# yjxiong/action-detection

Measured on NVIDIA H100. Metric: proposals/sec (9-seg BNInception SSN fwd+bwd), higher is better.
Workload: dtype f32 via split f16 operands (hi+lo, 3 wgmma MMAs per product) / f32 accumulate; f32 storage

## Files before the change

action-detection_b200/csrc/common.cuh:

```cuda
#pragma once
#include <cuda_fp16.h>
#include <cuda_runtime.h>
#include <stdint.h>

#include <atomic>
#include <string>

namespace ssnb {

struct View {
  void* base = nullptr;
  int H = 0, W = 0, C = 0, pitch = 0, coff = 0;
  long long lo_off = 0;
};

extern std::atomic<long long> g_launches;
void set_thread_error(const std::string& s);
const std::string& thread_error();

struct LaunchTag {
  int phase = 3;
  double flop = 0.0;
  const char* op = nullptr;
  int tiles = 0, block_n = 0;
};
extern thread_local bool t_timing;
extern thread_local LaunchTag t_tag;
void timing_mark(const char* what, cudaStream_t s);

#define SSNB_LAUNCH_CHECK(what)                                                       \
  do {                                                                                \
    ssnb::g_launches.fetch_add(1, std::memory_order_relaxed);                         \
    cudaError_t _e = cudaGetLastError();                                              \
    if (_e != cudaSuccess) {                                                          \
      ssnb::set_thread_error(std::string(what) + ": " + cudaGetErrorString(_e));      \
      return 2;                                                                       \
    }                                                                                 \
    if (ssnb::t_timing) ssnb::timing_mark(what, s);                                   \
  } while (0)

template <typename T> __device__ __forceinline__ float to_f(T v);
template <> __device__ __forceinline__ float to_f<float>(float v) { return v; }
template <> __device__ __forceinline__ float to_f<__half>(__half v) { return __half2float(v); }
template <typename T> __device__ __forceinline__ T from_f(float v);
template <> __device__ __forceinline__ float from_f<float>(float v) { return v; }
template <> __device__ __forceinline__ __half from_f<__half>(float v) { return __float2half_rn(v); }
__device__ __forceinline__ float relu(float v) { return v <= 0.f ? 0.f : v; }

constexpr float HALF_MAX = 65504.f;
__device__ __forceinline__ void split2(float a, float b, uint32_t& hi, uint32_t& lo) {
  const __half2 h = __floats2half2_rn(a, b);
  const float2 hf = __half22float2(h);
  const __half2 l = __floats2half2_rn(a - hf.x, b - hf.y);
  hi = *reinterpret_cast<const uint32_t*>(&h);
  lo = *reinterpret_cast<const uint32_t*>(&l);
}
__device__ __forceinline__ void store_planes4(__half* hi, long long lo_off, const float4& v) {
  uint2 h, l;
  split2(v.x, v.y, h.x, l.x);
  split2(v.z, v.w, h.y, l.y);
  *reinterpret_cast<uint2*>(hi) = h;
  *reinterpret_cast<uint2*>(reinterpret_cast<char*>(hi) + lo_off) = l;
}

struct ConvArgs {
  const void* src; int SH, SW, Csrc, src_pitch, src_coff;
  void* dst;       int DH, DW, Cdst, dst_pitch, dst_coff;
  const void* wgt;
  const float* bias;
  int F, kh, kw, stride, pad_h, pad_w;
  int relu, accumulate, dgrad;
};
struct WgradArgs {
  const void* dz; int OH, OW, Cout, dz_pitch, dz_coff;
  const void* x;  int IH, IW, Cin, x_pitch, x_coff;
  float* partial;
  int F, k, stride, pad, rows_per_split, splits;
};
template <typename T> int launch_conv(const ConvArgs& a, cudaStream_t s);
template <typename T> int launch_wgrad(const WgradArgs& a, cudaStream_t s);
int launch_wgrad_finalize(const float* partial, int splits, int taps, int Cout, int Cin, const float* mult,
                          float out_scale, float* dw_ref, int accumulate, cudaStream_t s, const float* bias_partial = nullptr,
                          float* db = nullptr, int* flag = nullptr,
                          const float* unscale = nullptr);

template <typename T> int launch_nchw_to_nhwc(const float* src, int F, int C, int H, int W, View dst, float scale, cudaStream_t s);
template <typename T> int launch_nhwc_to_nchw(View src, int F, float scale, float* dst, cudaStream_t s);
template <typename T> int launch_gpool_fwd(View src, int F, float* feat, cudaStream_t s);
template <typename T> int launch_gpool_bwd(const float* dfeat, float scale, const float* scale_dev, View ddst, int F, const void* y,
                                           cudaStream_t s);
constexpr int GRAD_EXP_TOP = 8, GRAD_EXP_MAX = 100;
int launch_grad_exponent(const float* dfeat, long long n, float grad_scale, int HW, float* gscale, int* flag, cudaStream_t s);

constexpr int PACK_MAX = 32;
constexpr int PACK_PER_THREAD = 4;
constexpr int PACK_TILE = 32, PACK_TILE_TAPS = 9;
inline int pack_ctas(int cout, int cin, int taps) {
  if (taps <= PACK_TILE_TAPS) return ((cout + PACK_TILE - 1) / PACK_TILE) * ((cin + PACK_TILE - 1) / PACK_TILE);
  const long long n = (long long)cout * cin * taps, per = 256LL * PACK_PER_THREAD;
  return (int)(((n > cout ? n : cout) + per - 1) / per);
}
struct PackEntry {
  const float *w, *b, *gamma, *beta, *mean, *var;
  void *wf, *wd; float *bias, *scale, *absmax;
  int cout, cin, taps, block0;
  int nofold, pad_[3];
  float* bias_b;
};
struct PackTable { int n, pad_; PackEntry e[PACK_MAX]; };
template <typename T> int launch_pack_all(const PackTable& t, int total_blocks, cudaStream_t s);
struct SplitEntry {
  const float *wf, *wd; __half *wf16, *wd16; long long plane_bytes, n; const float* absmax; float* inv_scale; int block0, pad_;
  __half *wd16_b, *wf16_b; long long b_plane_bytes; int b_pitch, cout;
};
struct SplitTable { int n, pad_; SplitEntry e[PACK_MAX]; };
int launch_split_all(const SplitTable& t, int total_blocks, cudaStream_t s);

constexpr int FIN_MAX = 36;
struct FinalizeEntry {
  const float* partial; const float* mult; float* dw; const float* bias_partial; float* db;
  int splits, taps, Cout, Cin, block0, pad_;
};
struct FinalizeTable { int n, total_blocks; int* flag; const float* unscale; FinalizeEntry e[FIN_MAX]; };
int launch_wgrad_finalize_all(const FinalizeTable& t, float out_scale, int accumulate, cudaStream_t s);

template <typename T> constexpr int VEC_WIDTH = 16 / (int)sizeof(T);
template <typename T>
int launch_maxpool_fwd_vec(View src, View dst, View dst_planes, int F, int k, int stride, int pad, uint8_t* argmax, cudaStream_t s);
template <typename T>
int launch_maxpool_bwd_vec(View dsrc, View ddst, int F, int k, int stride, int pad, const uint8_t* argmax, int accumulate, cudaStream_t s);
template <typename T> int launch_avgpool3_vec(View src, View dst, View dst_planes, int F, int accumulate, cudaStream_t s);
template <typename T>
int launch_mask_bias_vec(View dy, View y, View planes, float scale, int write_back, int* flag, int F, const float* mult, float out_scale,
                         const float* unscale, float* partial, int max_ctas, float* db, int accumulate, cudaStream_t s);
template <typename T>
int launch_pool_mask_bias_vec(View dz, View y, View dpool, View planes, float scale, int write_back, int* flag, int F, int k, int stride, int pad,
                              const uint8_t* argmax, const float* mult, float out_scale, const float* unscale, float* partial, int max_ctas,
                              float* db, int accumulate, cudaStream_t s);
int launch_split_view(View src_f32, int F, float scale, View planes, int* flag, cudaStream_t s);
int launch_planes_to_nchw(View planes, int F, float scale, float* dst, cudaStream_t s);
int launch_bn_train_fwd(View z, View y, View y_planes, int F, const float* gamma, const float* beta, float eps, float momentum, float* running_mean,
                        float* running_var, float* stat, float* partial, int max_ctas, cudaStream_t s);
int launch_bn_train_bwd(View z, View dy, View y, View dz, View dz_planes, float plane_scale, int* flag, int F, const float* gamma, float* stat,
                        float* partial, int max_ctas, float* dgamma, float* dbeta, const float* unscale, int accumulate, cudaStream_t s);
int launch_nhwc_to_s2d(View src, int F, __half* dst, long long lo_off, int Cs, cudaStream_t s);
int launch_nchw_to_s2d(const float* src, int F, int Cin, int H, int W, __half* dst, long long lo_off, int Cs, cudaStream_t s);
int launch_pack_conv1_s2d(const __half* wd, int Cout, int Cin, int Cs, __half* ws, cudaStream_t s);
int launch_wgrad_finalize_s2d(const float* partial, int splits, int Cout, int Cin, int Cs, const float* mult, float out_scale,
                              const float* unscale, float* dw_ref, int accumulate, cudaStream_t s);
int launch_upsample2_zero(View src, __half* dst, int H, int W, int F, cudaStream_t s);

}
```

action-detection_b200/csrc/engine.cu:

```cuda
#include <cstdio>
#include <cstdlib>
#include <algorithm>
#include <cstring>
#include <map>
#include <string>
#include <vector>

#include <cuda_profiler_api.h>

#include "../../include/ssnb.h"
#include "common.cuh"
#include "graph.cuh"
#include "umma_conv.cuh"

namespace ssnb {

std::atomic<long long> g_launches{0};
static thread_local std::string t_error;
void set_thread_error(const std::string& s) { t_error = s; }
const std::string& thread_error() { return t_error; }

thread_local bool t_timing = false;
thread_local LaunchTag t_tag;
struct TimingMark { const char* what; LaunchTag tag; std::string op; cudaEvent_t ev; };
static thread_local std::vector<TimingMark> t_marks;
static thread_local std::vector<cudaEvent_t> t_event_pool;
static thread_local std::string t_report;
static cudaEvent_t timing_event() {
  if (!t_event_pool.empty()) { cudaEvent_t e = t_event_pool.back(); t_event_pool.pop_back(); return e; }
  cudaEvent_t e = nullptr;
  cudaEventCreate(&e);
  return e;
}
void timing_mark(const char* what, cudaStream_t s) {
  TimingMark m{what, t_tag, t_tag.op ? t_tag.op : "", timing_event()};
  m.tag.op = nullptr;
  if (m.ev && cudaEventRecord(m.ev, s) == cudaSuccess) t_marks.push_back(m);
  else cudaGetLastError();
  t_tag.flop = 0.0; t_tag.op = nullptr; t_tag.tiles = 0; t_tag.block_n = 0;
}

static bool timing_close() {
  t_timing = false;
  if (t_marks.empty()) return false;
  if (cudaEventSynchronize(t_marks.back().ev) != cudaSuccess) { cudaGetLastError(); return false; }
  return true;
}

struct BlockSpec { const char* name; int c1, c3r, c3, cdr, cd1, cd2; int pool_max; int cproj; int stride; };
static const BlockSpec kBlocks[10] = {
    {"3a", 64, 64, 64, 64, 96, 96, 0, 32, 1},      {"3b", 64, 64, 96, 64, 96, 96, 0, 64, 1},
    {"3c", 0, 128, 160, 64, 96, 96, 1, 0, 2},      {"4a", 224, 64, 96, 96, 128, 128, 0, 128, 1},
    {"4b", 192, 96, 128, 96, 128, 128, 0, 128, 1}, {"4c", 160, 128, 160, 128, 160, 160, 0, 128, 1},
    {"4d", 96, 128, 192, 160, 192, 192, 0, 128, 1}, {"4e", 0, 128, 192, 192, 256, 256, 1, 0, 2},
    {"5a", 352, 192, 320, 160, 224, 224, 0, 128, 1}, {"5b", 352, 192, 320, 192, 224, 224, 1, 128, 1}};

static std::vector<Conv> conv_table(int in_ch) {
  std::vector<Conv> v;
  auto add = [&](const std::string& id, int cin, int cout, int k, int stride, int pad) { v.push_back({id, cin, cout, k, k, stride, pad, pad}); };
  add("conv1_7x7_s2", in_ch, 64, 7, 2, 3);
  add("conv2_3x3_reduce", 64, 64, 1, 1, 0);
  add("conv2_3x3", 64, 192, 3, 1, 1);
  int cx = 192;
  for (const BlockSpec& b : kBlocks) {
    std::string p = std::string("inception_") + b.name + "_";
    if (b.c1) add(p + "1x1", cx, b.c1, 1, 1, 0);
    add(p + "3x3_reduce", cx, b.c3r, 1, 1, 0);
    add(p + "3x3", b.c3r, b.c3, 3, b.stride, 1);
    add(p + "double_3x3_reduce", cx, b.cdr, 1, 1, 0);
    add(p + "double_3x3_1", b.cdr, b.cd1, 3, 1, 1);
    add(p + "double_3x3_2", b.cd1, b.cd2, 3, b.stride, 1);
    if (b.cproj) add(p + "pool_proj", cx, b.cproj, 1, 1, 0);
    cx = b.c1 + b.c3 + b.cd2 + (b.cproj ? b.cproj : cx);
  }
  return v;
}

struct Op : GraphOp {
  int grad_accumulate = 0;
  int wsplits = 1, wrows = 0;
  int tsplits = 1;
  size_t partial_off = 0, bias_partial_off = 0;
  UmmaConvPlan umma;
  UmmaConvPlan umma_dgrad;
  UmmaWgradPlan umma_wgrad;
  int pool_consumer = -1;
  bool folded_into_conv = false;
  bool dgrad_masks = false;
  bool bias_in_wgrad = false;
  bool dy_premasked = false;
  bool raw = false;
  int fuse_role = 0;
  int fuse_block = -1;
};
struct FusedBlock {
  int op1 = -1, op_r3 = -1, op_rd = -1;
  int c1 = 0, c3r = 0, cdr = 0, cx = 0;
  size_t w_fwd = 0, bias = 0, w_dg = 0;
  size_t w_fwd_plane = 0, w_dg_plane = 0, wmax = 0;
  UmmaConvPlan fwd, dgrad;
  bool enabled = false;
};

}

using namespace ssnb;

struct ssnb_engine : ssnb::Graph<ssnb::Op> {
  ssnb_config cfg;
  size_t up_plane = 0, s2d_plane = 0, s2d_w_plane = 0;
  int* tc_flag = nullptr;
  size_t tc_flag_off = 0;
  float* gscale = nullptr;
  bool bn1_train = false;
  const float *bn1_gamma = nullptr, *bn1_beta = nullptr; float *bn1_rmean = nullptr, *bn1_rvar = nullptr, *bn1_dgamma = nullptr, *bn1_dbeta = nullptr;
  float bn1_momentum = 0.1f, bn1_eps = 1e-5f;
  size_t bn_stat_off = 0, bn_partial_off = 0;
  std::vector<FusedBlock> fused;
  size_t ws_bytes = 0, partial_off = 0, partial_bytes = 0, bpartial_off = 0;
  size_t s2d_off = 0, s2d_w_off = 0, up_off = 0;
  bool fold_pools = true;
  bool s2d_ready = false;
  int Cs = 0;
  int conv1_tsplits = 128;
  bool weights_ready = false;
  std::vector<float*> dw, db;
  std::vector<int> pending_finalize;
  int grad_accumulate = 0;
  std::string error;
  long long launches0 = 0;
  UmmaContext umma_ctx;

  int fail(int code, const std::string& msg) { error = msg; return code; }
  const float* grad_scale_dev() const { return tensor_cores() ? gscale : nullptr; }
  const float* grad_unscale_dev() const { return tensor_cores() ? gscale + 1 : nullptr; }
  int nplanes() const { return exact_tc() ? 2 : 1; }
  const __half* w_fwd(const PackedConv& p) const { return (const __half*)(ws + (exact_tc() ? p.wd16 : p.wd)); }
  const __half* w_dgrad(const PackedConv& p) const { return (const __half*)(ws + (exact_tc() ? p.wf16 : p.wf)); }
  const UmmaTcOpts* tc_opts(UmmaTcOpts& t, size_t w_lo_off, void* out32, float alpha, size_t wmax) const {
    if (!exact_tc()) return nullptr;
    t.w_lo_off = (long long)w_lo_off; t.out32 = (float*)out32; t.alpha = alpha; t.alpha_dev = (const float*)(ws + wmax) + 1;
    return &t;
  }
};

namespace ssnb {

static bool profiled_op(const char* env, const std::string& id) {
  const char* e = getenv(env);
  if (!e || !*e) return false;
  const std::string list = std::string(",") + e + ",";
  return list.find("," + id + ",") != std::string::npos;
}
static bool env_on(const char* name) {
  const char* v = getenv(name);
  return v && v[0] == '1';
}
static int device_sms() {
  int dev = 0, sms = 0;
  if (cudaGetDevice(&dev) != cudaSuccess || cudaDeviceGetAttribute(&sms, cudaDevAttrMultiProcessorCount, dev) != cudaSuccess || sms <= 0) {
    cudaGetLastError();
    return 132;
  }
  return sms;
}

static void build_graph(ssnb_engine* e) {
  const int cin = e->cfg.in_channels;
  e->convs = conv_table(cin);
  int ci = 0;
  auto conv_op = [&](int in, int out) {
    const Conv& c = e->convs[ci];
    Op o; o.kind = OP_CONV; o.id = c.id; o.in = in; o.out = out; o.conv = ci;
    o.k = c.kh; o.stride = c.stride; o.pad = c.ph;
    e->ops.push_back(o);
    ++ci;
  };
  auto pool_op = [&](OpKind kind, const std::string& id, int in, int out, int k, int s, int p) {
    Op o; o.kind = kind; o.id = id; o.in = in; o.out = out; o.k = k; o.stride = s; o.pad = p;
    e->ops.push_back(o);
  };
  int x = e->whole("data", 224, 224, cin);
  int v;
  if (e->bn1_train) {
    const int raw = e->whole("conv1_7x7_s2_raw", 112, 112, 64); conv_op(x, raw); e->ops.back().raw = true;
    v = e->whole("conv1_7x7_s2_bn", 112, 112, 64);
    pool_op(OP_BN1, "conv1_7x7_s2_bn", raw, v, 0, 1, 0); x = v;
  } else {
    v = e->whole("conv1_7x7_s2_bn", 112, 112, 64); conv_op(x, v); x = v;
  }
  v = e->whole("pool1_3x3_s2", 56, 56, 64); pool_op(OP_MAXPOOL, "pool1_3x3_s2", x, v, 3, 2, 0); x = v;
  v = e->whole("conv2_3x3_reduce_bn", 56, 56, 64); conv_op(x, v); x = v;
  v = e->whole("conv2_3x3_bn", 56, 56, 192); conv_op(x, v); x = v;
  v = e->whole("pool2_3x3_s2", 28, 28, 192); pool_op(OP_MAXPOOL, "pool2_3x3_s2", x, v, 3, 2, 0); x = v;
  int H = 28, cx = 192;
  for (const BlockSpec& b : kBlocks) {
    const std::string p = std::string("inception_") + b.name + "_";
    const int OHW = (b.stride == 2) ? pool_out(H, 3, 2, 0) : H;
    const int ctot = b.c1 + b.c3 + b.cd2 + (b.cproj ? b.cproj : cx);
    const int cat = e->add_buffer(p + "output", OHW, OHW, ctot);
    const int red = e->add_buffer(p + "reduce", H, H, b.c3r + b.cdr);
    int off = 0;
    if (b.c1) { v = e->add_value(p + "1x1_bn", cat, off, b.c1); conv_op(x, v); off += b.c1; }
    int r3 = e->add_value(p + "3x3_reduce_bn", red, 0, b.c3r); conv_op(x, r3);
    v = e->add_value(p + "3x3_bn", cat, off, b.c3); conv_op(r3, v); off += b.c3;
    int rd = e->add_value(p + "double_3x3_reduce_bn", red, b.c3r, b.cdr); conv_op(x, rd);
    int d1 = e->whole(p + "double_3x3_1_bn", H, H, b.cd1); conv_op(rd, d1);
    v = e->add_value(p + "double_3x3_2_bn", cat, off, b.cd2); conv_op(d1, v); off += b.cd2;
    if (b.stride == 2) {
      v = e->add_value(p + "pool", cat, off, cx);
      pool_op(OP_MAXPOOL, p + "pool", x, v, 3, 2, 0);
    } else {
      int pl = e->whole(p + "pool", H, H, cx);
      pool_op(b.pool_max ? OP_MAXPOOL : OP_AVGPOOL, p + "pool", x, pl, 3, 1, 1);
      v = e->add_value(p + "pool_proj_bn", cat, off, b.cproj); conv_op(pl, v);
    }
    x = e->add_value(p + "output", cat, 0, ctot);
    H = OHW; cx = ctot;
  }
  Op g; g.kind = OP_GPOOL; g.id = "global_pool"; g.in = x; g.out = -1; g.k = 7;
  e->ops.push_back(g);
}

static void plan(ssnb_engine* e) {
  const size_t F = (size_t)e->F;
  size_t off = 0;
  e->tc_flag_off = off; off = align_up(off + 256, 1024);
  if (e->bn1_train) { e->bn_stat_off = off; off = align_up(off + 4 * 64 * 4, 1024); e->bn_partial_off = off; off = align_up(off + (size_t)1200 * 2 * 64 * 4, 1024); }
  off = e->plan_storage(off, e->cfg.training != 0, e->convs[0].cin, 16);
  size_t pmax = 0;
  if (e->cfg.training) {
    std::vector<char> written(e->vals.size(), 0);
    for (int i = (int)e->ops.size() - 1; i >= 0; --i) {
      Op& o = e->ops[i];
      o.grad_accumulate = written[o.in];
      written[o.in] = 1;
      if (o.kind == OP_CONV) {
        const Conv& c = e->convs[o.conv];
        const Buffer& ob = e->bufs[e->vals[o.out].buf];
        const long long M = (long long)F * ob.H * ob.W;
        const int taps = c.kh * c.kw;
        const bool flat = c.cin < 16;
        const long long tiles = (long long)((c.cout + 63) / 64) * (flat ? (taps * c.cin + 63) / 64 : ((c.cin + 63) / 64) * taps);
        long long splits = (592 + tiles - 1) / tiles;
        if (splits > 128) splits = 128;
        while (splits > 1 && M / splits < 256) --splits;
        long long rows = (M + splits - 1) / splits;
        rows = (rows + 15) / 16 * 16;
        splits = (M + rows - 1) / rows;
        o.wsplits = (int)splits; o.wrows = (int)rows;
        {
          const int chunks = (c.cin + 63) / 64, n_tiles = (chunks + 3) / 4, block_n = ((chunks + n_tiles - 1) / n_tiles) * 64;
          const int tpc = std::max(1, 4 / (block_n / 64));
          const int ctas = ((c.cout + 127) / 128) * n_tiles * ((taps + tpc - 1) / tpc);
          o.tsplits = std::max(o.wsplits, std::min(128, umma_wgrad_splits(ctas, umma_wgrad_ptiles(ob.W, ob.H, e->F), device_sms())));
        }
        if (e->tensor_cores()) splits = std::max<long long>(splits, o.tsplits);
        const size_t need = (size_t)splits * taps * c.cout * c.cin * 4;
        if (need > pmax) pmax = need;
      }
    }
  }
  if (e->tensor_cores()) {
    for (int i = 0; i < (int)e->ops.size(); ++i) {
      const Op& o = e->ops[i];
      if (o.kind != OP_CONV || o.k != 1) continue;
      const std::string& id = o.id;
      const std::string suf = "_3x3_reduce";
      if (id.size() < suf.size() || id.compare(id.size() - suf.size(), suf.size(), suf) != 0 || id.find("double") != std::string::npos) continue;
      const std::string pre = id.substr(0, id.size() - suf.size() + 1);
      FusedBlock fb; fb.op_r3 = i;
      for (int j = 0; j < (int)e->ops.size(); ++j) {
        if (e->ops[j].id == pre + "1x1") fb.op1 = j;
        if (e->ops[j].id == pre + "double_3x3_reduce") fb.op_rd = j;
      }
      if (fb.op_rd < 0) continue;
      fb.cx = e->convs[o.conv].cin; fb.c3r = e->convs[o.conv].cout; fb.cdr = e->convs[e->ops[fb.op_rd].conv].cout;
      fb.c1 = fb.op1 >= 0 ? e->convs[e->ops[fb.op1].conv].cout : 0;
      const int n = fb.c1 + fb.c3r + fb.cdr, kf = (fb.c1 + 63) / 64 * 64 + fb.c3r + fb.cdr;
      fb.w_fwd_plane = align_up((size_t)n * fb.cx * 2, 1024); fb.w_dg_plane = align_up((size_t)fb.cx * kf * 2, 1024);
      if (e->exact_tc()) fb.w_fwd_plane = fb.w_dg_plane = std::max(fb.w_fwd_plane, fb.w_dg_plane);
      fb.w_fwd = off; off += e->nplanes() * fb.w_fwd_plane;
      fb.bias = off; off = align_up(off + (size_t)n * 4, 256);
      fb.w_dg = off; off += e->nplanes() * fb.w_dg_plane;
      if (e->exact_tc()) {
        if (e->fused.size() >= 16) continue;
        fb.wmax = e->wmax_off + (e->convs.size() + e->fused.size()) * 8;
        for (int j : {fb.op1, fb.op_r3, fb.op_rd}) if (j >= 0) e->packed[e->ops[j].conv].wmax = fb.wmax;
      }
      e->fused.push_back(fb);
    }
  }
  if (e->tensor_cores()) {
    for (int i = 0; i < (int)e->ops.size(); ++i) {
      Op& po = e->ops[i];
      if (po.kind != OP_MAXPOOL || po.k != 3 || po.stride != 2 || po.pad != 0) continue;
      int producer = -1, consumers = 0;
      for (int j = 0; j < (int)e->ops.size(); ++j) {
        if (e->ops[j].out == po.in && e->ops[j].kind == OP_CONV) producer = j;
        if (e->ops[j].in == po.in) ++consumers;
      }
      if (producer >= 0 && consumers == 1 && e->vals[po.in].C % (e->fast() ? VEC_WIDTH<__half> : VEC_WIDTH<float>) == 0) { e->ops[producer].pool_consumer = i; po.folded_into_conv = true; }
    }
    auto operand_region = [&](size_t bytes, size_t& plane) {
      const size_t at = off;
      if (e->exact_tc()) { plane = align_up(bytes, 1024); off += 2 * plane; }
      else off = align_up(off + bytes, 1024);
      return at;
    };
    e->Cs = (4 * e->cfg.in_channels + 7) / 8 * 8;
    {
      const int chunks = (4 * e->Cs + 63) / 64, n_tiles = (chunks + 3) / 4, block_n = ((chunks + n_tiles - 1) / n_tiles) * 64;
      const int tpc = std::min(4, std::max(1, 4 / (block_n / 64)));
      const int ptiles = umma_wgrad_ptiles(112, 112, e->F);
      if ((ptiles + UMMA_WGRAD_MAX_PTILES - 1) / UMMA_WGRAD_MAX_PTILES > 128)
        e->conv1_tsplits = umma_wgrad_splits(n_tiles * ((4 + tpc - 1) / tpc), ptiles, device_sms());
    }
    e->s2d_off = operand_region(F * 112 * 112 * 4 * e->Cs * 2, e->s2d_plane);
    e->s2d_w_off = operand_region((size_t)16 * 64 * e->Cs * 2, e->s2d_w_plane);
    if (e->cfg.training) {
      size_t up = 0;
      for (const Op& o : e->ops)
        if (o.kind == OP_CONV && o.stride == 2 && o.conv != 0) {
          const Buffer& ib = e->bufs[e->vals[o.in].buf];
          up = std::max(up, F * ib.H * ib.W * (size_t)e->convs[o.conv].cout * 2);
        }
      e->up_off = operand_region(up, e->up_plane);
      pmax = std::max(pmax, (size_t)e->conv1_tsplits * 16 * 64 * e->Cs * 4);
    }
  }
  e->partial_off = off; e->partial_bytes = pmax; off = align_up(off + pmax, 1024);
  if (e->cfg.training)
    for (Op& o : e->ops)
      if (o.kind == OP_CONV) {
        const Conv& c = e->convs[o.conv];
        const int nsplit = e->tensor_cores() ? std::max(o.wsplits, o.tsplits) : o.wsplits;
        size_t need = (size_t)nsplit * c.kh * c.kw * c.cout * c.cin * 4;
        if (o.conv == 0 && e->tensor_cores()) need = std::max(need, (size_t)e->conv1_tsplits * 16 * 64 * e->Cs * 4);
        o.partial_off = off; off = align_up(off + need, 1024);
        o.bias_partial_off = off; off = align_up(off + (size_t)std::max(nsplit, 128) * c.cout * 4, 256);
      }
  e->bpartial_off = off; off = align_up(off + (size_t)1024 * 512 * 4, 1024);
  e->ws_bytes = off;
}

#define DISPATCH(e, call_f, call_h) ((e)->fast() ? (call_h) : (call_f))

static inline void tag_next(int phase, double flop, const char* op = nullptr) { t_tag.phase = phase; t_tag.flop = flop; t_tag.op = op; }
static thread_local std::string t_fused_name;
static const char* fused_name(const ssnb_engine* e, const FusedBlock& fb) {
  if (!t_timing) return nullptr;
  t_fused_name.clear();
  for (int j : {fb.op1, fb.op_r3, fb.op_rd})
    if (j >= 0) t_fused_name += (t_fused_name.empty() ? "" : "+") + e->ops[j].id;
  return t_fused_name.c_str();
}

static int run_fwd(ssnb_engine* e, const Op& o, float* feat, int n, cudaStream_t s) {
  tag_next(0, 0.0);
  if (o.kind == OP_CONV && o.umma.enabled) {
    if (o.conv == 0 && !e->s2d_ready) {
      const View in = e->view(o.in, false);
      __half* s2d = (__half*)(e->ws + e->s2d_off);
      if (int rc = launch_nhwc_to_s2d(in, n, s2d, (long long)e->s2d_plane, e->Cs, s)) return rc;
    }
    tag_next(0, e->conv_flops(o, n), o.id.c_str());
    return umma_conv_launch(e->umma_ctx, o.umma, s, false, n);
  }
  if (o.kind == OP_BN1) {
    if (!e->bn1_gamma || !e->bn1_beta) { set_thread_error("bn1_train engine: call ssnb_set_bn1 first"); return SSNB_ESTATE; }
    return launch_bn_train_fwd(e->view(o.in, false), e->view(o.out, false), e->exact_tc() ? e->planes(o.out, false) : View(), e->F, e->bn1_gamma,
                               e->bn1_beta, e->bn1_eps, e->bn1_momentum, e->bn1_rmean, e->bn1_rvar, (float*)(e->ws + e->bn_stat_off),
                               (float*)(e->ws + e->bn_partial_off), 1200, s);
  }
  if (o.kind == OP_MAXPOOL || o.kind == OP_AVGPOOL) return e->pool_fwd(o, n, s);
  if (o.kind == OP_GPOOL) {
    if (!feat) return e->fail(SSNB_EINVAL, "global_pool needs the feat output pointer");
    return e->gpool_fwd(o, n, feat, s);
  }
  if (int rc = e->simt_conv_fwd(o, o.raw ? 0 : 1, n, s)) return rc;
  if (!e->exact_tc() || !e->bufs[e->vals[o.out].buf].plane) return 0;
  return launch_split_view(e->view(o.out), n, 1.0f, e->planes(o.out), nullptr, s);
}

static int simt_wgrad(ssnb_engine* e, const Op& o, cudaStream_t s) {
  const Conv& c = e->convs[o.conv];
  const View x = e->view(o.in, false), dz = e->view(o.out, true);
  float* partial = (float*)(e->ws + o.partial_off);
  WgradArgs w;
  w.dz = dz.base; w.OH = dz.H; w.OW = dz.W; w.Cout = dz.C; w.dz_pitch = dz.pitch; w.dz_coff = dz.coff;
  w.x = x.base; w.IH = x.H; w.IW = x.W; w.Cin = x.C; w.x_pitch = x.pitch; w.x_coff = x.coff;
  w.partial = partial; w.F = e->F; w.k = c.kh; w.stride = c.stride; w.pad = c.ph;
  w.rows_per_split = o.wrows; w.splits = o.wsplits;
  tag_next(2, e->conv_flops(o, e->F), o.id.c_str());
  if (int rc = DISPATCH(e, launch_wgrad<float>(w, s), launch_wgrad<__half>(w, s))) return rc;
  const float out_scale = e->fast() ? 1.0f / e->cfg.grad_scale : 1.0f;
  return launch_wgrad_finalize(partial, o.wsplits, c.kh * c.kw, c.cout, c.cin, (const float*)(e->ws + e->packed[o.conv].scale), out_scale,
                               e->dw[o.conv], e->grad_accumulate, s, nullptr, nullptr, nullptr, e->grad_unscale_dev());
}
static int simt_dgrad(ssnb_engine* e, const Op& o, cudaStream_t s) {
  const Conv& c = e->convs[o.conv];
  const View dz = e->view(o.out, true), dx = e->view(o.in, true);
  ConvArgs a;
  a.src = dz.base; a.SH = dz.H; a.SW = dz.W; a.Csrc = dz.C; a.src_pitch = dz.pitch; a.src_coff = dz.coff;
  a.dst = dx.base; a.DH = dx.H; a.DW = dx.W; a.Cdst = dx.C; a.dst_pitch = dx.pitch; a.dst_coff = dx.coff;
  a.wgt = e->ws + e->packed[o.conv].wd; a.bias = nullptr;
  a.F = e->F; a.kh = a.kw = c.kh; a.stride = c.stride; a.pad_h = a.pad_w = c.ph; a.relu = 0; a.accumulate = o.grad_accumulate; a.dgrad = 1;
  tag_next(1, e->conv_flops(o, e->F), o.id.c_str());
  return DISPATCH(e, launch_conv<float>(a, s), launch_conv<__half>(a, s));
}

static int run_bwd(ssnb_engine* e, const Op& o, const float* dfeat, cudaStream_t s, bool skip_dgrad = false, bool full = false) {
  const int F = e->F;
  const float gs = e->fast() ? e->cfg.grad_scale : 1.0f;
  int rc = 0;
  tag_next(3, 0.0);
  if (o.kind == OP_GPOOL) {
    if (!dfeat) return e->fail(SSNB_EINVAL, "global_pool backward needs dfeat");
    const View din = e->view(o.in, true);
    const void* ym = (full && e->fold_pools && o.dgrad_masks) ? e->view(o.in, false).base : nullptr;
    const float* gsd = e->grad_scale_dev();
    return DISPATCH(e, launch_gpool_bwd<float>(dfeat, gs, gsd, din, F, ym, s), launch_gpool_bwd<__half>(dfeat, gs, gsd, din, F, ym, s));
  }
  if (o.kind == OP_BN1) {
    return launch_bn_train_bwd(e->view(o.in, false), e->view(o.out, true), e->view(o.out, false), e->view(o.in, true),
                               e->exact_tc() ? e->planes(o.in, true) : View(), e->cfg.grad_scale, e->tc_flag, F, e->bn1_gamma, (float*)(e->ws + e->bn_stat_off),
                               (float*)(e->ws + e->bn_partial_off), 1200, e->bn1_dgamma, e->bn1_dbeta, e->grad_unscale_dev(), e->grad_accumulate, s);
  }
  if (o.kind == OP_MAXPOOL) {
    if (full && e->fold_pools && o.folded_into_conv) return 0;
    const View din = e->view(o.in, true), dout = e->view(o.out, true);
    const uint8_t* am = (const uint8_t*)(e->ws + o.argmax_off);
    return DISPATCH(e, launch_maxpool_bwd_vec<float>(din, dout, F, o.k, o.stride, o.pad, am, o.grad_accumulate, s),
                    launch_maxpool_bwd_vec<__half>(din, dout, F, o.k, o.stride, o.pad, am, o.grad_accumulate, s));
  }
  if (o.kind == OP_AVGPOOL) {
    const View din = e->view(o.in, true), dout = e->view(o.out, true);
    return DISPATCH(e, launch_avgpool3_vec<float>(dout, din, View(), F, o.grad_accumulate, s),
                    launch_avgpool3_vec<__half>(dout, din, View(), F, o.grad_accumulate, s));
  }
  const Conv& c = e->convs[o.conv];
  const View x = e->view(o.in, false), y = e->view(o.out, false), dy = e->view(o.out, true);
  const float* scale = (const float*)(e->ws + e->packed[o.conv].scale);
  float* bpartial = (float*)(e->ws + e->bpartial_off);
  float* dbp = (e->db.size() && e->db[o.conv]) ? e->db[o.conv] : nullptr;
  const bool want_w = e->dw.size() && e->dw[o.conv];
  const bool want_x = e->vals[o.in].name != "data" && !skip_dgrad;
  const float gst = e->cfg.grad_scale;
  const float* us = e->grad_unscale_dev();
  const bool tc_w = want_w && o.umma_wgrad.enabled, tc_x = want_x && o.umma_dgrad.enabled;
  const bool pre = full && e->fold_pools && o.dy_premasked;
  const bool bias_w = pre && o.bias_in_wgrad && dbp && tc_w;
  const Op* pool = (full && e->fold_pools && o.pool_consumer >= 0) ? &e->ops[o.pool_consumer] : nullptr;
  const int max_ctas = (1024 * 512 - 64) / y.C;
  const View dpool = pool ? e->view(pool->out, true) : View();
  const uint8_t* pam = pool ? (const uint8_t*)(e->ws + pool->argmax_off) : nullptr;
  if (e->fast()) {
    if (pool) rc = launch_pool_mask_bias_vec<__half>(dy, y, dpool, View(), 1.0f, 1, nullptr, F, pool->k, pool->stride, pool->pad, pam,
                                                    scale, 1.0f / gst, us, bpartial, max_ctas, dbp, e->grad_accumulate, s);
    else if (!bias_w) rc = launch_mask_bias_vec<__half>(dy, pre ? View() : y, View(), 1.0f, 1, nullptr, F, scale, 1.0f / gst, us, bpartial, max_ctas, dbp,
                                                       e->grad_accumulate, s);
  } else {
    const bool need_f32 = (want_w && !tc_w) || (want_x && !tc_x);
    const View pl = (tc_w || tc_x) ? e->planes(o.out, true) : View();
    if (o.raw) {
      if (dbp) rc = launch_mask_bias_vec<float>(dy, View(), View(), gst, 0, nullptr, F, scale, 1.0f, us, bpartial, max_ctas, dbp, e->grad_accumulate, s);
    } else if (pre) {
      if (!bias_w && dbp) rc = launch_mask_bias_vec<float>(dy, y, View(), gst, 0, nullptr, F, scale, 1.0f, us, bpartial, max_ctas, dbp, e->grad_accumulate, s);
    } else if (pool) {
      rc = launch_pool_mask_bias_vec<float>(dy, y, dpool, pl, gst, need_f32 ? 1 : 0, e->tc_flag, F, pool->k, pool->stride, pool->pad, pam,
                                            scale, 1.0f, us, bpartial, max_ctas, dbp, e->grad_accumulate, s);
    } else {
      rc = launch_mask_bias_vec<float>(dy, y, pl, gst, (need_f32 || !full) ? 1 : 0, e->tc_flag, F, scale, 1.0f, us, bpartial, max_ctas, dbp,
                                       e->grad_accumulate, s);
    }
  }
  if (rc) return rc;
  if (tc_x && c.stride == 2 && o.conv != 0) {
    View dz = e->operand(o.out, true);
    for (int p = 0; p < e->nplanes(); ++p, dz.base = (char*)dz.base + dz.lo_off)
      if ((rc = launch_upsample2_zero(dz, (__half*)(e->ws + e->up_off + p * e->up_plane), x.H, x.W, F, s))) return rc;
  }
  if (tc_w) {
    float* partial = (float*)(e->ws + o.partial_off);
    float* bp = bias_w ? (float*)(e->ws + o.bias_partial_off) : nullptr;
    tag_next(2, e->conv_flops(o, F), o.id.c_str());
    if ((rc = umma_wgrad_launch(e->umma_ctx, o.umma_wgrad, s, bp))) return rc;
    if (full && o.conv != 0) e->pending_finalize.push_back((int)(&o - e->ops.data()));
    else if (o.conv == 0) rc = launch_wgrad_finalize_s2d(partial, o.umma_wgrad.p.splits, c.cout, c.cin, e->Cs, scale, 1.0f / gst, us, e->dw[o.conv],
                                                         e->grad_accumulate, s);
    else rc = launch_wgrad_finalize(partial, o.umma_wgrad.p.splits, c.kh * c.kw, c.cout, c.cin, scale, 1.0f / gst, e->dw[o.conv], e->grad_accumulate, s,
                                    nullptr, nullptr, e->tc_flag, us);
    if (rc) return rc;
  } else if (want_w && (rc = simt_wgrad(e, o, s))) return rc;
  if (tc_x) {
    tag_next(1, e->conv_flops(o, F), o.id.c_str());
    return umma_conv_launch(e->umma_ctx, o.umma_dgrad, s, full && e->fold_pools && o.dgrad_masks);
  }
  return want_x ? simt_dgrad(e, o, s) : 0;
}

int engine_tail_view(ssnb_handle h, View* v, int* F, int* fp16) {
  if (!h->ws || !h->weights_ready) return h->fail(SSNB_ESTATE, "workspace/weights not set");
  *v = h->view(h->ops.back().in, false);
  *F = h->F; *fp16 = h->fast() ? 1 : 0;
  return 0;
}

}

extern "C" {

const char* ssnb_version(void) { return "libssn_b200 0.3 (sm_90a)"; }

const char* ssnb_last_error(ssnb_handle h) { return h ? h->error.c_str() : ssnb::thread_error().c_str(); }

int ssnb_num_convs(void) { return 69; }

int ssnb_conv_info(int idx, int in_channels, char* name, int name_cap, int* cin, int* cout, int* k, int* stride, int* pad) {
  std::vector<Conv> t = conv_table(in_channels);
  if (idx < 0 || idx >= (int)t.size()) { set_thread_error("ssnb_conv_info: index out of range"); return SSNB_EINVAL; }
  if (name && name_cap > 0) { snprintf(name, name_cap, "%s", t[idx].id.c_str()); }
  if (cin) *cin = t[idx].cin; if (cout) *cout = t[idx].cout; if (k) *k = t[idx].kh;
  if (stride) *stride = t[idx].stride; if (pad) *pad = t[idx].ph;
  return SSNB_OK;
}

int ssnb_create(const ssnb_config* cfg, ssnb_handle* out) {
  if (!cfg || !out) { set_thread_error("ssnb_create: null argument"); return SSNB_EINVAL; }
  if (cfg->frames <= 0 || cfg->in_channels <= 0 || cfg->in_channels > 64) { set_thread_error("ssnb_create: bad frames/in_channels"); return SSNB_EINVAL; }
  if (cfg->precision != SSNB_EXACT_FP32 && cfg->precision != SSNB_FAST_FP16 && cfg->precision != SSNB_EXACT_TC) { set_thread_error("ssnb_create: unknown precision"); return SSNB_EINVAL; }
  ssnb_engine* e = new ssnb_engine();
  e->cfg = *cfg;
  if (!(e->cfg.grad_scale > 0.f)) e->cfg.grad_scale = 1.0f;
  e->F = cfg->frames;
  e->precision = cfg->precision;
  e->bn1_train = cfg->bn1_train != 0;
  if (e->bn1_train && e->fast()) { delete e; set_thread_error("ssnb_create: bn1_train (bn_mode='partial') needs EXACT_FP32 or EXACT_TC"); return SSNB_ENOSUPPORT; }
  e->esz = e->fast() ? 2 : 4;
  build_graph(e);
  if ((int)e->convs.size() != 69) { delete e; set_thread_error("internal: conv table size"); return SSNB_ESTATE; }
  umma_context_init(e->umma_ctx);
  plan(e);
  e->launches0 = g_launches.load();
  *out = e;
  return SSNB_OK;
}

int ssnb_destroy(ssnb_handle h) {
  if (!h) return SSNB_OK;
  umma_context_destroy(h->umma_ctx);
  delete h;
  return SSNB_OK;
}

size_t ssnb_workspace_bytes(ssnb_handle h) { return h ? h->ws_bytes : 0; }

int ssnb_set_workspace(ssnb_handle h, void* dev_ptr, size_t bytes) {
  if (!h) return SSNB_EINVAL;
  if (!dev_ptr || bytes < h->ws_bytes) return h->fail(SSNB_EINVAL, "workspace too small");
  if (((uintptr_t)dev_ptr) % 1024) return h->fail(SSNB_EINVAL, "workspace must be 1024-byte aligned");
  h->ws = (char*)dev_ptr;
  h->weights_ready = false;
  if (cudaMemset(h->ws + h->bpartial_off, 0, 256) != cudaSuccess) { cudaGetLastError();  }
  h->tc_flag = (int*)(h->ws + h->tc_flag_off);
  if (cudaMemset(h->tc_flag, 0, 256) != cudaSuccess) cudaGetLastError();
  h->gscale = (float*)(h->ws + h->tc_flag_off + 16);
  const float one[2] = {1.0f, 1.0f};
  if (cudaMemcpy(h->gscale, one, sizeof one, cudaMemcpyHostToDevice) != cudaSuccess) cudaGetLastError();
  const bool training = h->cfg.training != 0;
  const bool use_tc = h->tensor_cores() && !env_on("SSNB_DISABLE_UMMA");
  const bool use_wgrad = use_tc && training && !env_on("SSNB_DISABLE_UMMA_WGRAD");
  const bool fuse = !env_on("SSNB_DISABLE_FUSION");
  const float gs = h->cfg.grad_scale;
  for (Op& o : h->ops) {
    o.umma.enabled = o.umma_dgrad.enabled = o.umma_wgrad.enabled = false;
    o.fuse_role = 0; o.fuse_block = -1; o.dgrad_masks = o.dy_premasked = o.bias_in_wgrad = false;
  }
  for (FusedBlock& fb : h->fused) fb.enabled = false;
  h->fold_pools = fuse && (h->fast() || (use_tc && training));
  auto tc_gate = [&](UmmaConvPlan& p) {
    if (h->exact_tc() && !p.p.tc_ok) p.enabled = false;
    return p.enabled;
  };
  for (Op& o : h->ops) {
    if (o.kind != OP_CONV || !use_tc) continue;
    const Conv& c = h->convs[o.conv];
    const PackedConv& pk = h->packed[o.conv];
    UmmaTcOpts tf, tg;
    int rc = 0;
    if (o.conv == 0) {
      const int Ck = 4 * h->Cs;
      View xs; xs.base = h->ws + h->s2d_off; xs.H = 112; xs.W = 112; xs.C = Ck; xs.pitch = Ck; xs.coff = 0; xs.lo_off = (long long)h->s2d_plane;
      int dy[4], dx[4];
      for (int t = 0; t < 4; ++t) { dy[t] = t - 2; dx[t] = 0; }
      rc = umma_conv_bind_taps(h->umma_ctx, o.umma, xs, h->operand(o.out, false), h->F, Ck, c.cout, 4, dy, dx, (const __half*)(h->ws + h->s2d_w_off),
                               (const float*)(h->ws + pk.bias), o.raw ? 0 : 1, h->tc_opts(tf, h->s2d_w_plane, h->view(o.out, false).base, 1.0f, pk.wmax));
      if (rc) return h->fail(rc, "conv1 bind: " + ssnb::thread_error());
      tc_gate(o.umma);
      if (use_wgrad && (rc = umma_wgrad_bind_taps(h->umma_ctx, o.umma_wgrad, h->operand(o.out, true), xs, h->F, Ck, c.cout, 4, dy, dx,
                                                  (float*)(h->ws + o.partial_off), h->conv1_tsplits)))
        return h->fail(rc, "conv1 wgrad bind: " + ssnb::thread_error());
      continue;
    }
    if (c.cin % 8 != 0 || c.kh * c.kw > UMMA_MAX_TAPS) continue;
    rc = umma_conv_bind_fwd(h->umma_ctx, o.umma, h->operand(o.in, false), h->operand(o.out, false), h->F, c.cin, c.cout, c.kh, c.ph,
                            c.stride, h->w_fwd(pk), (const float*)(h->ws + pk.bias), h->tc_opts(tf, pk.wplane, h->view(o.out, false).base, 1.0f, pk.wmax));
    if (rc) return h->fail(rc, "bind_fwd(" + c.id + "): " + ssnb::thread_error());
    if (!training) continue;
    const View in = h->view(o.in, false);
    View dz = h->operand(o.out, true);
    if (c.stride == 2) { dz.base = h->ws + h->up_off; dz.H = in.H; dz.W = in.W; dz.C = c.cout; dz.pitch = c.cout; dz.coff = 0; dz.lo_off = (long long)h->up_plane; }
    View dx = h->view(o.in, true);
    const UmmaTcOpts* og = h->tc_opts(tg, pk.wplane, dx.base, 1.0f / gs, pk.wmax);
    if (og) dx.base = nullptr;
    rc = umma_conv_bind_dgrad(h->umma_ctx, o.umma_dgrad, dz, dx, h->F, c.cin, c.cout, c.kh, c.ph, h->w_dgrad(pk), o.grad_accumulate, og);
    if (rc) return h->fail(rc, "bind_dgrad(" + c.id + "): " + ssnb::thread_error());
    tc_gate(o.umma_dgrad);
    if (use_wgrad && (rc = umma_wgrad_bind(h->umma_ctx, o.umma_wgrad, h->operand(o.out, true), h->operand(o.in, false), h->F, c.cin, c.cout,
                                           c.kh, c.ph, (float*)(h->ws + o.partial_off), o.tsplits, c.stride)))
      return h->fail(rc, "wgrad_bind(" + c.id + "): " + ssnb::thread_error());
  }
  for (size_t bi = 0; bi < h->fused.size() && use_tc && fuse; ++bi) {
    FusedBlock& fb = h->fused[bi];
    const Op& o3 = h->ops[fb.op_r3]; const Op& od = h->ops[fb.op_rd];
    if (!o3.umma.enabled || !od.umma.enabled) continue;
    const int nr = fb.c3r + fb.cdr;
    const View x = h->operand(o3.in, false);
    View red = h->operand(o3.out, false); red.C = nr;
    UmmaTcOpts tf, tg;
    int rc;
    if (fb.op1 >= 0) {
      const int v1 = h->ops[fb.op1].out;
      const UmmaTcOpts* of = h->tc_opts(tf, fb.w_fwd_plane, h->view(v1, false).base, 1.0f, fb.wmax);
      tf.out32_2 = (float*)h->view(o3.out, false).base;
      rc = umma_conv_bind_fused_fwd(h->umma_ctx, fb.fwd, x, h->operand(v1, false), red, h->F, fb.cx, fb.c1, nr, (const __half*)(h->ws + fb.w_fwd),
                                    (const float*)(h->ws + fb.bias), of);
    } else {
      rc = umma_conv_bind_fwd(h->umma_ctx, fb.fwd, x, red, h->F, fb.cx, nr, 1, 0, 1, (const __half*)(h->ws + fb.w_fwd), (const float*)(h->ws + fb.bias),
                              h->tc_opts(tf, fb.w_fwd_plane, h->view(o3.out, false).base, 1.0f, fb.wmax));
    }
    if (rc) return h->fail(rc, "fused fwd bind(" + o3.id + "): " + ssnb::thread_error());
    if (!tc_gate(fb.fwd)) continue;
    if (training) {
      View dred = h->operand(o3.out, true); dred.C = nr;
      const View d1 = fb.op1 >= 0 ? h->operand(h->ops[fb.op1].out, true) : dred;
      View dx = h->view(o3.in, true);
      const UmmaTcOpts* og = h->tc_opts(tg, fb.w_dg_plane, dx.base, 1.0f / gs, fb.wmax);
      if (og) dx.base = nullptr;
      rc = umma_conv_bind_fused_dgrad(h->umma_ctx, fb.dgrad, d1, dred, dx, h->F, fb.cx, fb.c1, nr, (const __half*)(h->ws + fb.w_dg), od.grad_accumulate, og);
      if (rc) return h->fail(rc, "fused dgrad bind(" + o3.id + "): " + ssnb::thread_error());
      if (!tc_gate(fb.dgrad)) continue;
      if (h->exact_tc() && cudaMemset(h->ws + fb.w_dg, 0, 2 * fb.w_dg_plane) != cudaSuccess) cudaGetLastError();
    }
    fb.enabled = true;
    const int leader = fb.op1 >= 0 ? fb.op1 : fb.op_r3;
    for (int j : {fb.op1, fb.op_r3, fb.op_rd})
      if (j >= 0) { h->ops[j].fuse_block = (int)bi; h->ops[j].fuse_role = (j == leader) ? 1 : 2; }
  }
  if (use_tc && training && fuse) {
    std::vector<int> first_consumer(h->vals.size(), -1);
    for (int i = 0; i < (int)h->ops.size(); ++i)
      if (first_consumer[h->ops[i].in] < 0) first_consumer[h->ops[i].in] = i;
    for (size_t v = 0; v < h->vals.size(); ++v) {
      const int fc = first_consumer[v];
      if (fc < 0 || h->vals[v].name == "data") continue;
      if (h->exact_tc() && !h->bufs[h->vals[v].buf].plane) continue;
      bool conv_made = false;
      for (const Op& q : h->ops) conv_made = conv_made || (q.kind == OP_CONV && h->vals[q.out].buf == h->vals[v].buf);
      if (!conv_made) continue;
      Op& c = h->ops[fc];
      UmmaConvPlan* dg = nullptr;
      if (c.kind == OP_CONV && c.fuse_role == 1 && h->fused[c.fuse_block].enabled) dg = &h->fused[c.fuse_block].dgrad;
      else if (c.kind == OP_CONV && c.fuse_role == 0 && c.umma_dgrad.enabled) dg = &c.umma_dgrad;
      if (dg) {
        c.dgrad_masks = true;
        if (h->exact_tc()) {
          if (int rc = umma_conv_set_mask_tc(h->umma_ctx, *dg, h->view((int)v, false), h->planes((int)v, true), gs, h->tc_flag))
            return h->fail(rc, "mask bind(" + h->vals[v].name + "): " + ssnb::thread_error());
        } else {
          umma_conv_set_mask(*dg, h->view((int)v, false));
        }
      } else if (c.kind == OP_GPOOL && h->fast()) {
        c.dgrad_masks = true;
      }
    }
    for (Op& o : h->ops) {
      if (o.kind != OP_CONV) continue;
      int w = o.out;
      if (first_consumer[w] < 0) {
        const Value& ov = h->vals[o.out];
        for (size_t v = 0; v < h->vals.size(); ++v)
          if (h->vals[v].buf == ov.buf && h->vals[v].coff == 0 && h->vals[v].C == h->bufs[ov.buf].C && first_consumer[v] >= 0) { w = (int)v; break; }
      }
      if (first_consumer[w] >= 0 && h->ops[first_consumer[w]].dgrad_masks) o.dy_premasked = true;
      o.bias_in_wgrad = o.dy_premasked && o.conv != 0 && o.umma_wgrad.enabled;
    }
  }
  return SSNB_OK;
}

int ssnb_pack_weights(ssnb_handle h, const float* const* w, const float* const* b, const float* const* gamma,
                      const float* const* beta, const float* const* mean, const float* const* var, void* stream) {
  if (!h || !h->ws) return h ? h->fail(SSNB_ESTATE, "set_workspace first") : SSNB_EINVAL;
  cudaStream_t s = (cudaStream_t)stream;
  struct Member { int block = -1, row = 0, col = 0; };
  std::vector<Member> member(h->convs.size());
  for (size_t bi = 0; bi < h->fused.size(); ++bi) {
    const FusedBlock& fb = h->fused[bi];
    if (!fb.enabled) continue;
    const int k1p = (fb.c1 + 63) / 64 * 64;
    int row = 0, col = 0;
    for (int j : {fb.op1, fb.op_r3, fb.op_rd}) {
      if (j < 0) continue;
      const int ci = h->ops[j].conv;
      member[ci].block = (int)bi; member[ci].row = row; member[ci].col = col;
      row += h->convs[ci].cout;
      col += (j == fb.op1) ? k1p : h->convs[ci].cout;
    }
  }
  auto adjust = [&](size_t i, PackEntry& q, SplitEntry* e) {
    q.nofold = (h->bn1_train && i == 0) ? 1 : 0;
    const Member& mb = member[i];
    if (!h->exact_tc() || mb.block < 0) return;
    const FusedBlock& fb = h->fused[mb.block];
    q.bias_b = (float*)(h->ws + fb.bias) + mb.row;
    const int kf = (fb.c1 + 63) / 64 * 64 + fb.c3r + fb.cdr;
    e->wd16_b = (__half*)(h->ws + fb.w_fwd) + (size_t)mb.row * fb.cx;
    e->wf16_b = (__half*)(h->ws + fb.w_dg) + mb.col;
    e->b_pitch = kf;
    e->b_plane_bytes = (long long)std::max(fb.w_fwd_plane, fb.w_dg_plane);
  };
  if (int rc = h->pack_weights(w, b, gamma, beta, mean, var, h->convs[0].cin, adjust, "pack_weights", s)) return h->fail(rc, ssnb::thread_error());
  if (h->ops.size() && h->ops[0].umma.enabled) {
    const PackedConv& p = h->packed[0];
    for (int pl = 0; pl < h->nplanes(); ++pl) {
      int rc = launch_pack_conv1_s2d((const __half*)((const char*)h->w_fwd(p) + pl * p.wplane), h->convs[0].cout, h->convs[0].cin, h->Cs,
                                     (__half*)(h->ws + h->s2d_w_off + pl * h->s2d_w_plane), s);
      if (rc) return h->fail(rc, "pack conv1 s2d: " + ssnb::thread_error());
    }
  }
  for (FusedBlock& fb : h->fused) {
    if (!fb.enabled || !h->fast()) continue;
    const int k1p = (fb.c1 + 63) / 64 * 64, kf = k1p + fb.c3r + fb.cdr;
    __half* wfwd = (__half*)(h->ws + fb.w_fwd); float* bias = (float*)(h->ws + fb.bias); __half* wdg = (__half*)(h->ws + fb.w_dg);
    if (cudaMemsetAsync(wdg, 0, (size_t)fb.cx * kf * 2, s) != cudaSuccess) return h->fail(SSNB_ECUDA, "fused pack: memset");
    int row = 0, col = 0;
    for (int j : {fb.op1, fb.op_r3, fb.op_rd}) {
      if (j < 0) { continue; }
      const int ci = h->ops[j].conv, co = h->convs[ci].cout;
      cudaError_t e1 = cudaMemcpyAsync(wfwd + (size_t)row * fb.cx, h->ws + h->packed[ci].wd, (size_t)co * fb.cx * 2, cudaMemcpyDeviceToDevice, s);
      cudaError_t e2 = cudaMemcpyAsync(bias + row, h->ws + h->packed[ci].bias, (size_t)co * 4, cudaMemcpyDeviceToDevice, s);
      cudaError_t e3 = cudaMemcpy2DAsync(wdg + col, (size_t)kf * 2, h->ws + h->packed[ci].wf, (size_t)co * 2, (size_t)co * 2, fb.cx,
                                         cudaMemcpyDeviceToDevice, s);
      if (e1 != cudaSuccess || e2 != cudaSuccess || e3 != cudaSuccess) return h->fail(SSNB_ECUDA, "fused pack: copy failed");
      row += co;
      col += (j == fb.op1) ? k1p : co;
    }
  }
  h->weights_ready = true;
  return SSNB_OK;
}

int ssnb_set_bn1(ssnb_handle h, const float* gamma, const float* beta, float* running_mean, float* running_var, float* dgamma, float* dbeta,
                 float momentum, float eps) {
  if (!h) return SSNB_EINVAL;
  if (!h->bn1_train) return h->fail(SSNB_ESTATE, "engine created without bn1_train");
  if (!gamma || !beta) return h->fail(SSNB_EINVAL, "set_bn1: gamma / beta are required");
  h->bn1_gamma = gamma; h->bn1_beta = beta; h->bn1_rmean = running_mean; h->bn1_rvar = running_var; h->bn1_dgamma = dgamma; h->bn1_dbeta = dbeta;
  h->bn1_momentum = momentum; h->bn1_eps = eps;
  return SSNB_OK;
}

static int backbone_fwd(ssnb_handle h, const float* input_nchw, int n, float* feat, cudaStream_t s) {
  const View d = h->view(h->val_by_name["data"], false);
  int rc;
  h->s2d_ready = h->tensor_cores() && h->ops[0].umma.enabled;
  if (h->s2d_ready) rc = launch_nchw_to_s2d(input_nchw, n, d.C, d.H, d.W, (__half*)(h->ws + h->s2d_off), (long long)h->s2d_plane, h->Cs, s);
  else rc = h->value_write(h->val_by_name["data"], false, input_nchw, 1.0f, n, s);
  if (rc) { h->s2d_ready = false; return h->fail(rc, "input layout: " + ssnb::thread_error()); }
  for (size_t i = 0; i < h->ops.size(); ++i) {
    const Op& o = h->ops[i];
    if (o.fuse_role == 2) continue;
    const bool prof = profiled_op("SSNB_PROFILE_FWD_OPS", o.id);
    if (prof) cudaProfilerStart();
    int r;
    if (o.fuse_role == 1) {
      const FusedBlock& fb = h->fused[o.fuse_block];
      double fl = 0.0;
      for (int j : {fb.op1, fb.op_r3, fb.op_rd}) if (j >= 0) fl += h->conv_flops(h->ops[j], n);
      tag_next(0, fl, fused_name(h, fb));
      r = umma_conv_launch(h->umma_ctx, fb.fwd, s, false, n);
    } else r = run_fwd(h, o, feat, n, s);
    if (prof) cudaProfilerStop();
    if (r) { h->s2d_ready = false; return h->fail(r, "fwd " + o.id + ": " + ssnb::thread_error()); }
  }
  h->s2d_ready = false;
  return SSNB_OK;
}

int ssnb_backbone_fwd(ssnb_handle h, const float* input_nchw, float* feat, void* stream) {
  if (!h || !input_nchw || !feat) return h ? h->fail(SSNB_EINVAL, "null argument") : SSNB_EINVAL;
  if (!h->ws || !h->weights_ready) return h->fail(SSNB_ESTATE, "workspace/weights not set");
  return backbone_fwd(h, input_nchw, h->F, feat, (cudaStream_t)stream);
}

int ssnb_backbone_fwd_frames(ssnb_handle h, const float* input_nchw, int frames, float* feat, void* stream) {
  if (!h || !input_nchw || !feat) return h ? h->fail(SSNB_EINVAL, "null argument") : SSNB_EINVAL;
  if (frames < 1 || frames > h->F) return h->fail(SSNB_EINVAL, "backbone_fwd_frames: frames must be in 1 .. " + std::to_string(h->F));
  if (h->cfg.training) return h->fail(SSNB_ESTATE, "backbone_fwd_frames: runs forward-only engines (training = 0)");
  if (h->bn1_train) return h->fail(SSNB_ENOSUPPORT, "backbone_fwd_frames: bn1_train engines run their planned frame count only");
  if (!h->ws || !h->weights_ready) return h->fail(SSNB_ESTATE, "workspace/weights not set");
  return backbone_fwd(h, input_nchw, frames, feat, (cudaStream_t)stream);
}

int ssnb_bind_grads(ssnb_handle h, float* const* dw, float* const* db) {
  if (!h) return SSNB_EINVAL;
  h->dw.assign(h->convs.size(), nullptr); h->db.assign(h->convs.size(), nullptr);
  for (size_t i = 0; i < h->convs.size(); ++i) { if (dw) h->dw[i] = dw[i]; if (db) h->db[i] = db[i]; }
  return SSNB_OK;
}

int ssnb_backbone_bwd(ssnb_handle h, const float* dfeat, float* const* dw, float* const* db, void* stream) {
  return ssnb_backbone_bwd_range(h, dfeat, dw, db, -1, 0, stream);
}

int ssnb_backbone_bwd_range(ssnb_handle h, const float* dfeat, float* const* dw, float* const* db, int op_hi, int op_lo, void* stream) {
  if (!h || (!dfeat && (op_hi < 0 || op_hi >= (int)h->ops.size() - 1))) return h ? h->fail(SSNB_EINVAL, "null argument") : SSNB_EINVAL;
  if (!h->cfg.training) return h->fail(SSNB_ESTATE, "engine created without training=1");
  if (!h->ws || !h->weights_ready) return h->fail(SSNB_ESTATE, "workspace/weights not set");
  ssnb_bind_grads(h, dw, db);
  h->pending_finalize.clear();
  cudaStream_t s = (cudaStream_t)stream;
  auto run_range = [&](int hi, int lo) -> int {
    for (int i = hi; i >= lo; --i) {
      const Op& o = h->ops[i];
      const bool prof = profiled_op("SSNB_PROFILE_BWD_OPS", o.id);
      if (prof) cudaProfilerStart();
      int rc = run_bwd(h, o, dfeat, s, o.fuse_role != 0, true);
      if (!rc && o.fuse_role == 1) {
        const FusedBlock& fb = h->fused[o.fuse_block];
        double fl = 0.0;
        for (int j : {fb.op1, fb.op_r3, fb.op_rd}) if (j >= 0) fl += h->conv_flops(h->ops[j], h->F);
        tag_next(1, fl, fused_name(h, fb));
        rc = umma_conv_launch(h->umma_ctx, fb.dgrad, s, h->fold_pools && o.dgrad_masks);
      }
      if (prof) cudaProfilerStop();
      if (rc) return h->fail(rc, "bwd " + o.id + ": " + ssnb::thread_error());
    }
    return 0;
  };
  auto finalize = [&]() -> int {
    const float gs = h->tensor_cores() ? h->cfg.grad_scale : 1.0f;
    FinalizeTable t; t.n = 0; t.total_blocks = 0; t.flag = h->tc_flag; t.unscale = h->grad_unscale_dev();
    auto flush = [&]() -> int { int rc = launch_wgrad_finalize_all(t, 1.0f / gs, h->grad_accumulate, s); t.n = 0; t.total_blocks = 0; return rc; };
    for (int oi : h->pending_finalize) {
      const Op& o = h->ops[oi];
      const Conv& c = h->convs[o.conv];
      FinalizeEntry& q = t.e[t.n];
      q.partial = (const float*)(h->ws + o.partial_off); q.mult = (const float*)(h->ws + h->packed[o.conv].scale); q.dw = h->dw[o.conv];
      const bool bias_w = o.dy_premasked && o.bias_in_wgrad && h->db.size() && h->db[o.conv];
      q.bias_partial = bias_w ? (const float*)(h->ws + o.bias_partial_off) : nullptr; q.db = bias_w ? h->db[o.conv] : nullptr;
      q.splits = o.umma_wgrad.p.splits; q.taps = c.kh * c.kw; q.Cout = c.cout; q.Cin = c.cin; q.block0 = t.total_blocks; q.pad_ = 0;
      t.total_blocks += (int)(((long long)q.taps * q.Cout * q.Cin + 255) / 256);
      if (++t.n == FIN_MAX) if (int rc = flush()) { h->pending_finalize.clear(); return h->fail(rc, "finalize: " + ssnb::thread_error()); }
    }
    h->pending_finalize.clear();
    if (int rc = flush()) return h->fail(rc, "finalize: " + ssnb::thread_error());
    return 0;
  };
  const int last = (int)h->ops.size() - 1;
  if (op_hi < 0 || op_hi > last) op_hi = last;
  if (op_lo < 0 || op_lo > op_hi) return h->fail(SSNB_EINVAL, "backbone_bwd_range: bad op range");
  if (op_hi == last && h->tensor_cores()) {
    if (int rc = launch_grad_exponent(dfeat, (long long)h->F * h->vals[h->ops[last].in].C, h->cfg.grad_scale,
                                      h->bufs[h->vals[h->ops[last].in].buf].H * h->bufs[h->vals[h->ops[last].in].buf].W, h->gscale, h->tc_flag, s))
      return h->fail(rc, "gradient exponent: " + ssnb::thread_error());
  }
  if (int rc = run_range(op_hi, op_lo)) return rc;
  return finalize();
}

int ssnb_set_grad_accumulate(ssnb_handle h, int accumulate) {
  if (!h) return SSNB_EINVAL;
  h->grad_accumulate = accumulate ? 1 : 0;
  return SSNB_OK;
}

int ssnb_num_ops(ssnb_handle h) { return h ? (int)h->ops.size() : 0; }

int ssnb_op_info(ssnb_handle h, int op, char* kind, int kind_cap, char* in_name, int in_cap, char* out_name, int out_cap) {
  if (!h || op < 0 || op >= (int)h->ops.size()) return SSNB_EINVAL;
  const Op& o = h->ops[op];
  if (kind) snprintf(kind, kind_cap, "%s", kOpKindName[o.kind]);
  if (in_name) snprintf(in_name, in_cap, "%s", h->vals[o.in].name.c_str());
  if (out_name) snprintf(out_name, out_cap, "%s", o.out >= 0 ? h->vals[o.out].name.c_str() : "feat");
  return SSNB_OK;
}

int ssnb_value_shape(ssnb_handle h, const char* name, int* c, int* hh, int* ww) {
  if (!h || !name) return SSNB_EINVAL;
  const int v = h->value_of(name);
  if (v < 0) return h->fail(SSNB_EINVAL, std::string("unknown value ") + name);
  const View w = h->view(v, false);
  if (c) *c = w.C; if (hh) *hh = w.H; if (ww) *ww = w.W;
  return SSNB_OK;
}

static float host_gscale(ssnb_handle h, int which, cudaStream_t s) {
  float v = 1.0f;
  if (!h->tensor_cores() || cudaMemcpyAsync(&v, h->gscale + which, sizeof v, cudaMemcpyDeviceToHost, s) != cudaSuccess ||
      cudaStreamSynchronize(s) != cudaSuccess) { cudaGetLastError(); return 1.0f; }
  return v;
}

int ssnb_value_write(ssnb_handle h, const char* name, int grad, const float* src_nchw, void* stream) {
  if (!h || !name || !src_nchw || !h->ws) return SSNB_EINVAL;
  const int v = h->value_of(name);
  if (v < 0) return h->fail(SSNB_EINVAL, std::string("unknown value ") + name);
  if (grad && !h->cfg.training) return h->fail(SSNB_ESTATE, "no gradient buffers");
  const float sc = grad ? (h->fast() ? h->cfg.grad_scale : 1.0f) * host_gscale(h, 0, (cudaStream_t)stream) : 1.0f;
  const int rc = h->value_write(v, grad != 0, src_nchw, sc, h->F, (cudaStream_t)stream);
  return rc ? h->fail(rc, ssnb::thread_error()) : SSNB_OK;
}

int ssnb_value_read(ssnb_handle h, const char* name, int grad, float* dst_nchw, void* stream) {
  if (!h || !name || !dst_nchw || !h->ws) return SSNB_EINVAL;
  const int v = h->value_of(name);
  if (v < 0) return h->fail(SSNB_EINVAL, std::string("unknown value ") + name);
  if ((grad & 1) && !h->cfg.training) return h->fail(SSNB_ESTATE, "no gradient buffers");
  if (grad & 2) {
    if (!h->exact_tc() || !h->bufs[h->vals[v].buf].plane) return h->fail(SSNB_ESTATE, "value has no operand planes");
    const float sc = (grad & 1) ? host_gscale(h, 1, (cudaStream_t)stream) / h->cfg.grad_scale : 1.0f;
    const int rc = h->planes_read(v, (grad & 1) != 0, sc, dst_nchw, (cudaStream_t)stream);
    return rc ? h->fail(rc, ssnb::thread_error()) : SSNB_OK;
  }
  const float sc = grad ? host_gscale(h, 1, (cudaStream_t)stream) / (h->fast() ? h->cfg.grad_scale : 1.0f) : 1.0f;
  const int rc = h->value_read(v, grad != 0, sc, dst_nchw, (cudaStream_t)stream);
  return rc ? h->fail(rc, ssnb::thread_error()) : SSNB_OK;
}

int ssnb_run_op(ssnb_handle h, int op, int backward, void* stream) {
  if (!h || op < 0 || op >= (int)h->ops.size()) return SSNB_EINVAL;
  if (!h->ws || !h->weights_ready) return h->fail(SSNB_ESTATE, "workspace/weights not set");
  const Op& o = h->ops[op];
  if (o.kind == OP_GPOOL) return h->fail(SSNB_ENOSUPPORT, "run_op: global_pool runs through backbone_fwd/bwd");
  int rc = backward ? run_bwd(h, o, nullptr, (cudaStream_t)stream) : run_fwd(h, o, nullptr, h->F, (cudaStream_t)stream);
  return rc ? h->fail(rc, o.id + ": " + ssnb::thread_error()) : SSNB_OK;
}

int ssnb_grad_overflow(ssnb_handle h, int clear) {
  if (!h) return -1;
  if (!h->tc_flag) return 0;
  int v = 0;
  if (cudaMemcpy(&v, h->tc_flag, sizeof(int), cudaMemcpyDeviceToHost) != cudaSuccess) { cudaGetLastError(); return -1; }
  if (v && clear) cudaMemset(h->tc_flag, 0, sizeof(int));
  return v ? 1 : 0;
}

int ssnb_timing_begin(void* stream) {
  for (TimingMark& m : ssnb::t_marks) ssnb::t_event_pool.push_back(m.ev);
  ssnb::t_marks.clear();
  ssnb::t_tag = LaunchTag();
  ssnb::t_timing = true;
  ssnb::timing_mark("(begin)", (cudaStream_t)stream);
  return SSNB_OK;
}

const char* ssnb_timing_report(void) {
  ssnb::t_report.clear();
  if (!ssnb::timing_close()) return ssnb::t_report.c_str();
  struct Agg { int n = 0; double ms = 0, flop = 0; };
  std::map<std::pair<std::string, int>, Agg> agg;
  for (size_t i = 1; i < ssnb::t_marks.size(); ++i) {
    float ms = 0.f;
    if (cudaEventElapsedTime(&ms, ssnb::t_marks[i - 1].ev, ssnb::t_marks[i].ev) != cudaSuccess) { cudaGetLastError(); continue; }
    Agg& a = agg[{ssnb::t_marks[i].what, ssnb::t_marks[i].tag.phase}];
    a.n += 1; a.ms += ms; a.flop += ssnb::t_marks[i].tag.flop;
  }
  char line[256];
  for (const auto& kv : agg) {
    snprintf(line, sizeof line, "%s\t%d\t%d\t%.6f\t%.0f\n", kv.first.first.c_str(), kv.first.second, kv.second.n, kv.second.ms, kv.second.flop);
    ssnb::t_report += line;
  }
  return ssnb::t_report.c_str();
}

const char* ssnb_timing_launches(void) {
  ssnb::t_report.clear();
  if (!ssnb::timing_close()) return ssnb::t_report.c_str();
  char line[512];
  for (size_t i = 1; i < ssnb::t_marks.size(); ++i) {
    const ssnb::TimingMark& m = ssnb::t_marks[i];
    float ms = 0.f;
    if (cudaEventElapsedTime(&ms, ssnb::t_marks[i - 1].ev, m.ev) != cudaSuccess) { cudaGetLastError(); continue; }
    snprintf(line, sizeof line, "%s\t%d\t%s\t%.6f\t%.0f\t%d\t%d\n", m.what, m.tag.phase, m.op.empty() ? "-" : m.op.c_str(), ms, m.tag.flop,
             m.tag.tiles, m.tag.block_n);
    ssnb::t_report += line;
  }
  return ssnb::t_report.c_str();
}

int64_t ssnb_launch_count(ssnb_handle h) { return h ? (int64_t)(g_launches.load() - h->launches0) : 0; }
int64_t ssnb_global_launch_count(void) { return (int64_t)g_launches.load(); }

}
```

action-detection_b200/csrc/s2d_glue.cu:

```cuda
#include "common.cuh"

#include <type_traits>

namespace ssnb {
namespace {

template <typename T>
__global__ void nhwc_to_s2d_kernel(const T* __restrict__ src, int F, int H, int W, int Cin, int spitch, int scoff,
                                   __half* __restrict__ dst, long long lo_off, int Cs) {
  const int H2 = H / 2, W2 = W / 2, Ck = 4 * Cs;
  const long long total = (long long)F * H2 * W2 * Ck;
  const long long i = (long long)blockIdx.x * blockDim.x + threadIdx.x;
  if (i >= total) return;
  const int ch = (int)(i % Ck);
  const long long p = i / Ck;
  const int x2 = (int)(p % W2), y2 = (int)((p / W2) % H2);
  const long long f = p / ((long long)W2 * H2);
  const int ds = ch / Cs, q = ch % Cs;
  T v = 0.f;
  const int xs = x2 + ds - 2;
  if (q < 4 * Cin && xs >= 0 && xs < W2) {
    const int ab = q / Cin, c = q % Cin;
    v = src[((f * H + 2 * y2 + ab / 2) * W + 2 * xs + ab % 2) * spitch + scoff + c];
  }
  if constexpr (std::is_same_v<T, float>) {
    const __half h = __float2half_rn(v);
    dst[i] = h;
    *reinterpret_cast<__half*>(reinterpret_cast<char*>(dst + i) + lo_off) = __float2half_rn(v - __half2float(h));
  } else {
    dst[i] = v;
  }
}

__global__ void pack_conv1_s2d_kernel(const __half* __restrict__ wd, int Cout, int Cin, int Cs, __half* __restrict__ ws) {
  const int Ck = 4 * Cs;
  const long long total = (long long)4 * Cout * Ck;
  const long long i = (long long)blockIdx.x * blockDim.x + threadIdx.x;
  if (i >= total) return;
  const int ch = (int)(i % Ck);
  const int co = (int)((i / Ck) % Cout);
  const int dr = (int)(i / ((long long)Ck * Cout));
  const int ds = ch / Cs, q = ch % Cs;
  __half v = __float2half_rn(0.f);
  if (q < 4 * Cin) {
    const int ab = q / Cin, c = q % Cin;
    const int r = 2 * dr + ab / 2 - 1, s = 2 * ds + ab % 2 - 1;
    if (r >= 0 && r < 7 && s >= 0 && s < 7) v = wd[((long long)(r * 7 + s) * Cout + co) * Cin + c];
  }
  ws[i] = v;
}

__global__ void wgrad_finalize_s2d_kernel(const float* __restrict__ partial, int splits, int Cout, int Cin, int Cs,
                                          const float* __restrict__ mult, float out_scale, const float* __restrict__ unscale,
                                          float* __restrict__ dw, int accumulate) {
  const int Ck = 4 * Cs;
  const long long total = (long long)Cout * Cin * 49;
  const long long i = (long long)blockIdx.x * blockDim.x + threadIdx.x;
  if (i >= total) return;
  const int s = (int)(i % 7), r = (int)((i / 7) % 7);
  const int c = (int)((i / 49) % Cin), co = (int)(i / (49LL * Cin));
  const int dr = (r + 1) / 2, a = (r + 1) % 2, ds = (s + 1) / 2, b = (s + 1) % 2;
  const int ch = ds * Cs + (a * 2 + b) * Cin + c;
  float acc = 0.f;
  for (int sp = 0; sp < splits; ++sp) acc += partial[(((long long)sp * 4 + dr) * Cout + co) * Ck + ch];
  if (unscale) out_scale *= __ldg(unscale);
  dw[i] = (accumulate ? dw[i] : 0.f) + acc * mult[co] * out_scale;
}

template <int CS, int CIN, bool LO>
__global__ void nchw_to_s2d_kernel(const float* __restrict__ src, int F, int Cin_rt, int H, int W, __half* __restrict__ dst,
                                   long long lo_off) {
  const int Cin = CIN ? CIN : Cin_rt;
  const int H2 = H / 2, W2 = W / 2;
  const long long i = (long long)blockIdx.x * blockDim.x + threadIdx.x;
  if (i >= (long long)F * H2 * W2 * 4) return;
  const unsigned iu = (unsigned)i;
  const int ds = (int)(iu & 3u);
  const unsigned pu = iu >> 2;
  const int x2 = (int)(pu % (unsigned)W2), y2 = (int)((pu / (unsigned)W2) % (unsigned)H2);
  const long long p = pu;
  const long long f = pu / (unsigned)(W2 * H2);
  __align__(16) __half vh[CS];
  __align__(16) __half vl[LO ? CS : 1];
#pragma unroll
  for (int c = 0; c < CS; ++c) {
    vh[c] = __float2half_rn(0.f);
    if constexpr (LO) vl[c] = __float2half_rn(0.f);
  }
  const int xs = x2 + ds - 2;
  if (xs >= 0 && xs < W2) {
#pragma unroll
    for (int c = 0; c < Cin; ++c) {
      const float* pl = src + ((f * Cin + c) * H + 2 * y2) * (long long)W + 2 * xs;
      const float2 r0 = __ldg(reinterpret_cast<const float2*>(pl));
      const float2 r1 = __ldg(reinterpret_cast<const float2*>(pl + W));
      const float q[4] = {r0.x, r0.y, r1.x, r1.y};
#pragma unroll
      for (int ab = 0; ab < 4; ++ab) {
        const __half h = __float2half_rn(q[ab]);
        vh[ab * Cin + c] = h;
        if constexpr (LO) vl[ab * Cin + c] = __float2half_rn(q[ab] - __half2float(h));
      }
    }
  }
  __half* o = dst + p * (4 * CS) + ds * CS;
  uint4* oh = reinterpret_cast<uint4*>(o);
  uint4* ol = reinterpret_cast<uint4*>(reinterpret_cast<char*>(o) + lo_off);
#pragma unroll
  for (int q = 0; q < CS / 8; ++q) {
    oh[q] = reinterpret_cast<const uint4*>(vh)[q];
    if constexpr (LO) ol[q] = reinterpret_cast<const uint4*>(vl)[q];
  }
}

__global__ void upsample2_zero_kernel(const __half* __restrict__ src, int OH, int OW, int C, int spitch, int scoff,
                                      __half* __restrict__ dst, int H, int W, int F) {
  const int G = C / 8;
  const long long total = (long long)F * H * W * G;
  const long long i = (long long)blockIdx.x * blockDim.x + threadIdx.x;
  if (i >= total) return;
  const unsigned iu = (unsigned)i;
  const int g = (int)(iu % (unsigned)G);
  const unsigned pu = iu / (unsigned)G;
  const int x = (int)(pu % (unsigned)W), y = (int)((pu / (unsigned)W) % (unsigned)H);
  const long long p = pu;
  const long long f = pu / (unsigned)(W * H);
  uint4 v = make_uint4(0u, 0u, 0u, 0u);
  if (!(x & 1) && !(y & 1) && y / 2 < OH && x / 2 < OW)
    v = __ldg(reinterpret_cast<const uint4*>(src + ((f * OH + y / 2) * OW + x / 2) * spitch + scoff + g * 8));
  *reinterpret_cast<uint4*>(dst + p * C + g * 8) = v;
}

}

int launch_nhwc_to_s2d(View src, int F, __half* dst, long long lo_off, int Cs, cudaStream_t s) {
  const long long n = (long long)F * (src.H / 2) * (src.W / 2) * 4 * Cs;
  const unsigned g = (unsigned)((n + 255) / 256);
  if (lo_off) nhwc_to_s2d_kernel<float><<<g, 256, 0, s>>>((const float*)src.base, F, src.H, src.W, src.C, src.pitch, src.coff, dst, lo_off, Cs);
  else nhwc_to_s2d_kernel<__half><<<g, 256, 0, s>>>((const __half*)src.base, F, src.H, src.W, src.C, src.pitch, src.coff, dst, lo_off, Cs);
  SSNB_LAUNCH_CHECK("nhwc_to_s2d_kernel");
  return 0;
}
template <bool LO>
static int nchw_to_s2d(const float* src, int F, int Cin, int H, int W, __half* dst, long long lo_off, int Cs, cudaStream_t s) {
  const long long n = (long long)F * (H / 2) * (W / 2) * 4;
  const unsigned g = (unsigned)((n + 255) / 256);
  if (Cs == 16 && Cin == 3) nchw_to_s2d_kernel<16, 3, LO><<<g, 256, 0, s>>>(src, F, Cin, H, W, dst, lo_off);
  else if (Cs == 40 && Cin == 10) nchw_to_s2d_kernel<40, 10, LO><<<g, 256, 0, s>>>(src, F, Cin, H, W, dst, lo_off);
  else if (Cs == 16) nchw_to_s2d_kernel<16, 0, LO><<<g, 256, 0, s>>>(src, F, Cin, H, W, dst, lo_off);
  else if (Cs == 40) nchw_to_s2d_kernel<40, 0, LO><<<g, 256, 0, s>>>(src, F, Cin, H, W, dst, lo_off);
  else { set_thread_error("nchw_to_s2d: unsupported channel count (RGB 3 or Flow 10)"); return 1; }
  SSNB_LAUNCH_CHECK("nchw_to_s2d_kernel");
  return 0;
}
int launch_nchw_to_s2d(const float* src, int F, int Cin, int H, int W, __half* dst, long long lo_off, int Cs, cudaStream_t s) {
  return lo_off ? nchw_to_s2d<true>(src, F, Cin, H, W, dst, lo_off, Cs, s) : nchw_to_s2d<false>(src, F, Cin, H, W, dst, lo_off, Cs, s);
}
int launch_pack_conv1_s2d(const __half* wd, int Cout, int Cin, int Cs, __half* ws, cudaStream_t s) {
  const long long n = 16LL * Cout * Cs;
  pack_conv1_s2d_kernel<<<(unsigned)((n + 255) / 256), 256, 0, s>>>(wd, Cout, Cin, Cs, ws);
  SSNB_LAUNCH_CHECK("pack_conv1_s2d_kernel");
  return 0;
}
int launch_wgrad_finalize_s2d(const float* partial, int splits, int Cout, int Cin, int Cs, const float* mult, float out_scale,
                              const float* unscale, float* dw_ref, int accumulate, cudaStream_t s) {
  const long long n = (long long)Cout * Cin * 49;
  wgrad_finalize_s2d_kernel<<<(unsigned)((n + 255) / 256), 256, 0, s>>>(partial, splits, Cout, Cin, Cs, mult, out_scale, unscale, dw_ref, accumulate);
  SSNB_LAUNCH_CHECK("wgrad_finalize_s2d_kernel");
  return 0;
}
int launch_upsample2_zero(View src, __half* dst, int H, int W, int F, cudaStream_t s) {
  const long long n = (long long)F * H * W * (src.C / 8);
  upsample2_zero_kernel<<<(unsigned)((n + 255) / 256), 256, 0, s>>>((const __half*)src.base, src.H, src.W, src.C, src.pitch, src.coff, dst, H, W, F);
  SSNB_LAUNCH_CHECK("upsample2_zero_kernel");
  return 0;
}

}
```

action-detection_b200/csrc/umma_conv.cu:

```cuda
#include <cstdio>
#include <cstdlib>
#include <cstring>
#include <algorithm>

#include "umma_conv.cuh"
#include "umma_dev.cuh"

namespace ssnb {

namespace {

using namespace umma;
constexpr int MAX_STAGES = 8;
constexpr int PIPE_BYTES = 192 * 1024;
constexpr int A_BYTES = BLOCK_M * BLOCK_K * 2;
constexpr int NUM_THREADS = 384;
constexpr int N_STEP = 16;
constexpr int MAX_BLOCK_N = 128;
constexpr int EPI_COLS = 16;
constexpr int EPI_F32_BYTES = BLOCK_M * EPI_COLS * 4;
constexpr int EPI_F16_BYTES = BLOCK_M * EPI_COLS * 2;
constexpr int EPI_BYTES = EPI_F32_BYTES + 2 * EPI_F16_BYTES;
constexpr int BAR_BYTES = 256;
constexpr int SMEM_BYTES = PIPE_BYTES + 2 * EPI_BYTES + BAR_BYTES + 1024 ;
constexpr int ORDER_BAR = 1;
constexpr int EPI_BAR = 3;
static_assert(SMEM_BYTES <= 227 * 1024, "shared memory per block");

struct TileCoord { int w0, h0, f0, n0; };
__device__ __forceinline__ TileCoord decode_tile(const UmmaConvParams& p, int tile) {
  TileCoord t;
  const int nt = tile % p.n_tiles;
  int m = tile / p.n_tiles;
  t.n0 = nt * p.block_n;
  t.w0 = (m % p.tiles_w) * p.bw; m /= p.tiles_w;
  t.h0 = (m % p.tiles_h) * p.bh; m /= p.tiles_h;
  t.f0 = m * p.bf;
  return t;
}

__device__ __forceinline__ uint32_t sw64_off(int r, int c) { return r * 64 + ((((c >> 2) ^ (r >> 1)) & 3) << 4) + (c & 3) * 4; }
__device__ __forceinline__ uint32_t sw32_off(int r, int c) { return r * 32 + ((((c >> 3) ^ (r >> 2)) & 1) << 4) + (c & 7) * 2; }

__device__ __forceinline__ uint32_t h2_bits(__half2 h) { return *reinterpret_cast<const uint32_t*>(&h); }

template <int BN, int NK>
__device__ __forceinline__ void mma_k(float* d0, float* d1, uint32_t sa, uint32_t sb) {
#pragma unroll
  for (int k = 0; k < NK; ++k) {
    const uint64_t bdesc = make_desc_sw128(sb + k * MMA_K * 2);
    wgmma<BN, 0, 0>(d0, make_desc_sw128(sa + k * MMA_K * 2), bdesc);
    wgmma<BN, 0, 0>(d1, make_desc_sw128(sa + 64 * 128 + k * MMA_K * 2), bdesc);
  }
}

template <int BN, int NK>
__device__ __forceinline__ void mma_stage(float* d0, float* d1, uint32_t sa, uint32_t sb, uint32_t b_bytes, bool split) {
  if (split) {
    mma_k<BN, NK>(d0, d1, sa + A_BYTES, sb);
    mma_k<BN, NK>(d0, d1, sa, sb + b_bytes);
  }
  mma_k<BN, NK>(d0, d1, sa, sb);
}

__device__ __forceinline__ void ring_advance(uint32_t& stage, uint32_t& phase, int n, int stages) {
  const uint32_t s = stage + (uint32_t)n;
  phase ^= (s / (uint32_t)stages) & 1u;
  stage = s % (uint32_t)stages;
}

template <int BN, bool DIRECT>
__device__ __forceinline__ void
umma_conv_body(const CUtensorMap& tmap_a, const CUtensorMap& tmap_a2, const CUtensorMap& tmap_b, const CUtensorMap& tmap_a_lo,
               const CUtensorMap& tmap_a2_lo, const CUtensorMap& tmap_b_lo, const CUtensorMap& tmap_o, const CUtensorMap& tmap_o_hi,
               const CUtensorMap& tmap_o_lo, const CUtensorMap& tmap_o2, const CUtensorMap& tmap_o2_hi, const CUtensorMap& tmap_o2_lo,
               const UmmaConvParams& p) {
  extern __shared__ uint8_t smem_raw[];
  uint8_t* smem = reinterpret_cast<uint8_t*>((reinterpret_cast<uintptr_t>(smem_raw) + 1023) & ~(uintptr_t)1023);
  const int STAGES = p.stages, STAGE_BYTES = p.stage_bytes;
  uint64_t* bars = reinterpret_cast<uint64_t*>(smem + PIPE_BYTES + 2 * EPI_BYTES);
  uint64_t* full_bar = bars;
  uint64_t* empty_bar = bars + MAX_STAGES;

  const int wg = __shfl_sync(0xffffffffu, (int)threadIdx.x / 128, 0);
  const int total_tiles = p.tiles_w * p.tiles_h * p.tiles_f * p.n_tiles;
  const bool split = p.nseg > 1;
  const int nplanes = split ? 2 : 1;
  const uint32_t b_bytes = (uint32_t)p.block_n * BLOCK_K * 2;
  const int ksteps = p.ntaps * p.kchunks;

  if (threadIdx.x == 0) {
    asm volatile("prefetch.tensormap [%0];" ::"l"(reinterpret_cast<uint64_t>(&tmap_a)) : "memory");
    asm volatile("prefetch.tensormap [%0];" ::"l"(reinterpret_cast<uint64_t>(&tmap_a2)) : "memory");
    asm volatile("prefetch.tensormap [%0];" ::"l"(reinterpret_cast<uint64_t>(&tmap_b)) : "memory");
    asm volatile("prefetch.tensormap [%0];" ::"l"(reinterpret_cast<uint64_t>(&tmap_o)) : "memory");
    for (int i = 0; i < STAGES; ++i) { mbar_init(&full_bar[i], 1); mbar_init(&empty_bar[i], 1); }
    asm volatile("fence.mbarrier_init.release.cluster;" ::: "memory");
  }
  __syncthreads();

  if (wg == 0) {
    producer_regs();
    if (threadIdx.x == 0) {
      uint32_t stage = 0, phase = 0;
      const uint32_t a_bytes = (uint32_t)(p.bw * p.bh * p.bf) * BLOCK_K * 2;
      const uint32_t tx_bytes = (a_bytes + b_bytes) * nplanes;
      for (int tile = blockIdx.x; tile < total_tiles; tile += gridDim.x) {
        const TileCoord t = decode_tile(p, tile);
        for (int tap = 0; tap < p.ntaps; ++tap) {
          for (int kc = 0; kc < p.kchunks; ++kc) {
            mbar_wait(&empty_bar[stage], phase ^ 1);
            uint8_t* sa = smem + stage * STAGE_BYTES;
            uint8_t* sb = sa + nplanes * A_BYTES;
            mbar_expect_tx(&full_bar[stage], tx_bytes);
            for (int pl = 0; pl < nplanes; ++pl) {
              if (kc < p.kchunks_a1)
                tma_load_4d(sa + pl * A_BYTES, pl ? &tmap_a_lo : &tmap_a, &full_bar[stage], kc * BLOCK_K, t.w0 * p.a_stride + p.tap_dx[tap],
                            t.h0 * p.a_stride + p.tap_dy[tap], t.f0);
              else
                tma_load_4d(sa + pl * A_BYTES, pl ? &tmap_a2_lo : &tmap_a2, &full_bar[stage], (kc - p.kchunks_a1) * BLOCK_K, t.w0 + p.tap_dx[tap],
                            t.h0 + p.tap_dy[tap], t.f0);
              tma_load_3d(sb + pl * b_bytes, pl ? &tmap_b_lo : &tmap_b, &full_bar[stage], kc * BLOCK_K, t.n0, tap);
            }
            if (++stage == STAGES) { stage = 0; phase ^= 1; }
          }
        }
      }
    }
  } else {
    consumer_regs();
    const int cw = wg - 1, row = threadIdx.x & 127;
    const int warp = row / 32, lane = row & 31;
    uint8_t* epi = smem + PIPE_BYTES + cw * EPI_BYTES;
    const float alpha = p.out_f32 ? p.alpha * (p.alpha_dev ? __ldg(p.alpha_dev) : 1.0f) : 1.0f;
    const int my_tiles = (total_tiles - (int)blockIdx.x + (int)gridDim.x - 1) / (int)gridDim.x;
    uint32_t stage = 0, phase = 0;
    if (cw) ring_advance(stage, phase, ksteps, STAGES);
    for (int j = cw; j < my_tiles; j += 2) {
      const TileCoord t = decode_tile(p, (int)blockIdx.x + j * (int)gridDim.x);
      float acc[2][BN / 2];
#pragma unroll
      for (int b = 0; b < 2; ++b)
#pragma unroll
        for (int i = 0; i < BN / 2; ++i) acc[b][i] = 0.f;
      if (j > 0) named_bar_sync(ORDER_BAR + cw, 256);
      uint32_t prev = 0;
      int kc = 0;
      for (int ks = 0; ks < ksteps; ++ks) {
        mbar_wait(&full_bar[stage], phase);
        const uint32_t sa = smem_u32(smem + stage * STAGE_BYTES);
        const uint32_t sb = sa + nplanes * A_BYTES;
        const int kvalid = kc < p.kchunks_a1 ? p.K1 - kc * BLOCK_K : p.K - p.K1 - (kc - p.kchunks_a1) * BLOCK_K;
        const int nk = kvalid >= BLOCK_K ? BLOCK_K / MMA_K : (kvalid + MMA_K - 1) / MMA_K;
        wgmma_fence();
        switch (nk) {
          case 1: mma_stage<BN, 1>(acc[0], acc[1], sa, sb, b_bytes, split); break;
          case 2: mma_stage<BN, 2>(acc[0], acc[1], sa, sb, b_bytes, split); break;
          case 3: mma_stage<BN, 3>(acc[0], acc[1], sa, sb, b_bytes, split); break;
          default: mma_stage<BN, BLOCK_K / MMA_K>(acc[0], acc[1], sa, sb, b_bytes, split); break;
        }
        wgmma_commit();
        wgmma_wait<1>();
        if (ks > 0 && row == 0) mbar_arrive(&empty_bar[prev]);
        prev = stage;
        if (++stage == STAGES) { stage = 0; phase ^= 1; }
        if (++kc == p.kchunks) kc = 0;
      }
      if (j + 1 < my_tiles) named_bar_arrive(ORDER_BAR + (cw ^ 1), 256);
      wgmma_wait<0>();
      if (row == 0) mbar_arrive(&empty_bar[prev]);
      ring_advance(stage, phase, ksteps, STAGES);
      const bool direct = DIRECT && t.f0 >= p.f_direct;
      bool rv[2][2];
      int rpix[2][2];
#pragma unroll
      for (int b = 0; b < 2; ++b)
#pragma unroll
        for (int h = 0; h < 2; ++h) {
          const int r = b * 64 + warp * 16 + (lane >> 2) + 8 * h;
          const int rw = r % p.bw, rh = (r / p.bw) % p.bh, rf = r / (p.bw * p.bh);
          const int w = t.w0 + rw, y = t.h0 + rh, f = t.f0 + rf;
          rv[b][h] = rf < p.bf && w < p.W && y < p.H && f < p.F;
          rpix[b][h] = (f * p.H + y) * p.W + w;
        }
      const int q2 = 2 * (lane & 3);
#pragma unroll
      for (int sl = 0; sl < BN / EPI_COLS; ++sl) {
        const int col = t.n0 + sl * EPI_COLS;
        if (col >= p.Cout) break;
        const bool d1 = col < p.n_split;
        const int cd = d1 ? col : col - p.n_split;
        const int opitch = d1 ? p.out_pitch : p.out2_pitch, ocoff = d1 ? p.out_coff : p.out2_coff;
        float v[2][2][4];
#pragma unroll
        for (int b = 0; b < 2; ++b)
#pragma unroll
          for (int h = 0; h < 2; ++h)
#pragma unroll
            for (int k = 0; k < 2; ++k) {
              const int i = sl * (EPI_COLS / 2) + 4 * k + 2 * h;
              v[b][h][2 * k] = acc[b][i]; v[b][h][2 * k + 1] = acc[b][i + 1];
            }
        const bool planes = p.out_f32 && (d1 ? p.planes : p.planes2);
        if (p.out_f32) {
#pragma unroll
          for (int b = 0; b < 2; ++b)
#pragma unroll
            for (int h = 0; h < 2; ++h)
#pragma unroll
              for (int j = 0; j < 4; ++j) v[b][h][j] = __fmul_rn(v[b][h][j], alpha);
          if (p.bias) {
#pragma unroll
            for (int k = 0; k < 2; ++k) {
              const float2 bb = __ldg(reinterpret_cast<const float2*>(p.bias + col + 8 * k + q2));
#pragma unroll
              for (int b = 0; b < 2; ++b)
#pragma unroll
                for (int h = 0; h < 2; ++h) { v[b][h][2 * k] = __fadd_rn(v[b][h][2 * k], bb.x); v[b][h][2 * k + 1] = __fadd_rn(v[b][h][2 * k + 1], bb.y); }
            }
          }
          if (p.accumulate) {
            const float* o32 = (d1 ? p.out32 : p.out32_2) + ocoff + cd + q2;
#pragma unroll
            for (int b = 0; b < 2; ++b)
#pragma unroll
              for (int h = 0; h < 2; ++h)
                if (rv[b][h])
#pragma unroll
                  for (int k = 0; k < 2; ++k) {
                    const float2 o = *reinterpret_cast<const float2*>(o32 + (long long)rpix[b][h] * opitch + 8 * k);
                    v[b][h][2 * k] = __fadd_rn(v[b][h][2 * k], o.x); v[b][h][2 * k + 1] = __fadd_rn(v[b][h][2 * k + 1], o.y);
                  }
          }
          if (p.relu) {
#pragma unroll
            for (int b = 0; b < 2; ++b)
#pragma unroll
              for (int h = 0; h < 2; ++h)
#pragma unroll
                for (int j = 0; j < 4; ++j) v[b][h][j] = relu(v[b][h][j]);
          }
          if (p.mask32) {
            const float* m32 = p.mask32 + p.mask32_coff + col + q2;
#pragma unroll
            for (int b = 0; b < 2; ++b)
#pragma unroll
              for (int h = 0; h < 2; ++h)
#pragma unroll
                for (int k = 0; k < 2; ++k) {
                  const float2 y = rv[b][h] ? __ldg(reinterpret_cast<const float2*>(m32 + (long long)rpix[b][h] * p.mask32_pitch + 8 * k)) : make_float2(0.f, 0.f);
                  if (!(y.x > 0.f)) v[b][h][2 * k] = 0.f;
                  if (!(y.y > 0.f)) v[b][h][2 * k + 1] = 0.f;
                }
          }
        } else {
          if (p.bias) {
#pragma unroll
            for (int k = 0; k < 2; ++k) {
              const float2 bb = __ldg(reinterpret_cast<const float2*>(p.bias + col + 8 * k + q2));
#pragma unroll
              for (int b = 0; b < 2; ++b)
#pragma unroll
                for (int h = 0; h < 2; ++h) { v[b][h][2 * k] += bb.x; v[b][h][2 * k + 1] += bb.y; }
            }
          }
          if (p.accumulate) {
            const __half* o16 = (d1 ? p.out : p.out2) + ocoff + cd + q2;
#pragma unroll
            for (int b = 0; b < 2; ++b)
#pragma unroll
              for (int h = 0; h < 2; ++h)
                if (rv[b][h])
#pragma unroll
                  for (int k = 0; k < 2; ++k) {
                    const float2 o = __half22float2(*reinterpret_cast<const __half2*>(o16 + (long long)rpix[b][h] * opitch + 8 * k));
                    v[b][h][2 * k] += o.x; v[b][h][2 * k + 1] += o.y;
                  }
          }
          if (p.relu) {
#pragma unroll
            for (int b = 0; b < 2; ++b)
#pragma unroll
              for (int h = 0; h < 2; ++h)
#pragma unroll
                for (int j = 0; j < 4; ++j) v[b][h][j] = relu(v[b][h][j]);
          }
          if (p.mask_y) {
            const __half* my = p.mask_y + p.mask_coff + col + q2;
#pragma unroll
            for (int b = 0; b < 2; ++b)
#pragma unroll
              for (int h = 0; h < 2; ++h)
#pragma unroll
                for (int k = 0; k < 2; ++k) {
                  const float2 y = rv[b][h] ? __half22float2(__ldg(reinterpret_cast<const __half2*>(my + (long long)rpix[b][h] * p.mask_pitch + 8 * k)))
                                            : make_float2(0.f, 0.f);
                  if (!(y.x > 0.f)) v[b][h][2 * k] = 0.f;
                  if (!(y.y > 0.f)) v[b][h][2 * k + 1] = 0.f;
                }
          }
        }
        if (row == 0) bulk_wait_read0();
        named_bar_sync(EPI_BAR + cw, 128);
        const bool scaled = p.flag || p.plane_scale != 1.0f;
        float m = 0.f;
#pragma unroll
        for (int b = 0; b < 2; ++b)
#pragma unroll
          for (int h = 0; h < 2; ++h) {
            const int r = b * 64 + warp * 16 + (lane >> 2) + 8 * h;
            if (p.out_f32) {
              const bool s = (lane >> 3) & 1;
              const float2 x0 = make_float2(v[b][h][0], v[b][h][1]), x1 = make_float2(v[b][h][2], v[b][h][3]);
              *reinterpret_cast<float2*>(epi + sw64_off(r, q2 + (s ? 8 : 0))) = s ? x1 : x0;
              *reinterpret_cast<float2*>(epi + sw64_off(r, q2 + (s ? 0 : 8))) = s ? x0 : x1;
              if (planes)
#pragma unroll
                for (int k = 0; k < 2; ++k) {
                  float x0 = v[b][h][2 * k], x1 = v[b][h][2 * k + 1];
                  if (scaled) {
                    x0 = __fmul_rn(x0, p.plane_scale); x1 = __fmul_rn(x1, p.plane_scale);
                    if (rv[b][h]) {
                      m = fmaxf(m, fabsf(x0)); if (x0 != x0) m = INFINITY;
                      m = fmaxf(m, fabsf(x1)); if (x1 != x1) m = INFINITY;
                    }
                  }
                  const __half2 hh = __floats2half2_rn(x0, x1);
                  const float2 hf = __half22float2(hh);
                  *reinterpret_cast<uint32_t*>(epi + EPI_F32_BYTES + sw32_off(r, 8 * k + q2)) = h2_bits(hh);
                  *reinterpret_cast<uint32_t*>(epi + EPI_F32_BYTES + EPI_F16_BYTES + sw32_off(r, 8 * k + q2)) =
                      h2_bits(__floats2half2_rn(__fsub_rn(x0, hf.x), __fsub_rn(x1, hf.y)));
                }
            } else {
#pragma unroll
              for (int k = 0; k < 2; ++k)
                *reinterpret_cast<uint32_t*>(epi + sw32_off(r, 8 * k + q2)) = h2_bits(__floats2half2_rn(v[b][h][2 * k], v[b][h][2 * k + 1]));
            }
          }
        if (planes && p.flag && !(m <= 65504.f)) *p.flag = 1;
        fence_proxy_async_smem();
        named_bar_sync(EPI_BAR + cw, 128);
        if (row == 0 && !direct) {
          tma_store_4d(d1 ? &tmap_o : &tmap_o2, epi, cd, t.w0, t.h0, t.f0);
          if (planes) {
            tma_store_4d(d1 ? &tmap_o_hi : &tmap_o2_hi, epi + EPI_F32_BYTES, cd, t.w0, t.h0, t.f0);
            tma_store_4d(d1 ? &tmap_o_lo : &tmap_o2_lo, epi + EPI_F32_BYTES + EPI_F16_BYTES, cd, t.w0, t.h0, t.f0);
          }
          bulk_commit();
        }
        if (direct) {
          const int rw = row % p.bw, rh = (row / p.bw) % p.bh, rf = row / (p.bw * p.bh);
          const int w = t.w0 + rw, y = t.h0 + rh, f = t.f0 + rf;
          if (rf < p.bf && w < p.W && y < p.H && f < p.F) {
            const long long po = ((long long)(f * p.H + y) * p.W + w) * opitch + ocoff + cd;
            if (p.out_f32) {
              float* o32 = (d1 ? p.out32 : p.out32_2) + po;
#pragma unroll 1
              for (int j = 0; j < EPI_COLS / 4; ++j)
                *reinterpret_cast<float4*>(o32 + 4 * j) = *reinterpret_cast<const float4*>(epi + sw64_off(row, 4 * j));
            }
            if (!p.out_f32 || planes) {
              const uint8_t* st = epi + (p.out_f32 ? EPI_F32_BYTES : 0);
              char* o16 = reinterpret_cast<char*>((d1 ? p.out : p.out2) + po);
              const long long lo = d1 ? p.out_lo : p.out2_lo;
#pragma unroll 1
              for (int j = 0; j < EPI_COLS / 8; ++j) {
                *reinterpret_cast<uint4*>(o16 + 16 * j) = *reinterpret_cast<const uint4*>(st + sw32_off(row, 8 * j));
                if (planes) *reinterpret_cast<uint4*>(o16 + lo + 16 * j) = *reinterpret_cast<const uint4*>(st + EPI_F16_BYTES + sw32_off(row, 8 * j));
              }
            }
          }
        }
      }
    }
    if (row == 0) bulk_wait0();
  }
}

#define UMMA_CONV_PARAMS                                                                                                    \
  const __grid_constant__ CUtensorMap tmap_a, const __grid_constant__ CUtensorMap tmap_a2, const __grid_constant__ CUtensorMap tmap_b, \
      const __grid_constant__ CUtensorMap tmap_a_lo, const __grid_constant__ CUtensorMap tmap_a2_lo,                               \
      const __grid_constant__ CUtensorMap tmap_b_lo, const __grid_constant__ CUtensorMap tmap_o,                                   \
      const __grid_constant__ CUtensorMap tmap_o_hi, const __grid_constant__ CUtensorMap tmap_o_lo,                                \
      const __grid_constant__ CUtensorMap tmap_o2, const __grid_constant__ CUtensorMap tmap_o2_hi,                                 \
      const __grid_constant__ CUtensorMap tmap_o2_lo, const __grid_constant__ UmmaConvParams p
#define UMMA_CONV_ARGS tmap_a, tmap_a2, tmap_b, tmap_a_lo, tmap_a2_lo, tmap_b_lo, tmap_o, tmap_o_hi, tmap_o_lo, tmap_o2, tmap_o2_hi, tmap_o2_lo, p

template <int BN>
__global__ void __launch_bounds__(NUM_THREADS, 1) umma_conv_kernel(UMMA_CONV_PARAMS) { umma_conv_body<BN, false>(UMMA_CONV_ARGS); }
template <int BN>
__global__ void __launch_bounds__(NUM_THREADS, 1) umma_conv_tail_kernel(UMMA_CONV_PARAMS) { umma_conv_body<BN, true>(UMMA_CONV_ARGS); }

typedef CUresult (*EncodeTiledFn)(CUtensorMap*, CUtensorMapDataType, cuuint32_t, void*, const cuuint64_t*, const cuuint64_t*,
                                  const cuuint32_t*, const cuuint32_t*, CUtensorMapInterleave, CUtensorMapSwizzle,
                                  CUtensorMapL2promotion, CUtensorMapFloatOOBfill);

int resolve_encode(UmmaContext& ctx) {
  if (ctx.encode_tiled) return 0;
  void* fn = nullptr;
  cudaDriverEntryPointQueryResult q;
  cudaError_t e = cudaGetDriverEntryPoint("cuTensorMapEncodeTiled", &fn, cudaEnableDefault, &q);
  if (e != cudaSuccess || q != cudaDriverEntryPointSuccess || !fn) {
    cudaGetLastError();
    set_thread_error("cuTensorMapEncodeTiled not available from the driver");
    return 2;
  }
  ctx.encode_tiled = fn;
  int dev = 0, sms = 132;
  if (cudaGetDevice(&dev) == cudaSuccess) cudaDeviceGetAttribute(&sms, cudaDevAttrMultiProcessorCount, dev);
  ctx.num_sms = sms;
  return 0;
}

int encode(UmmaContext& ctx, CUtensorMap* m, int rank, void* addr, const cuuint64_t* dims, const cuuint64_t* strides,
           const cuuint32_t* box, int spatial_stride = 1, CUtensorMapDataType dtype = CU_TENSOR_MAP_DATA_TYPE_FLOAT16,
           CUtensorMapSwizzle swizzle = CU_TENSOR_MAP_SWIZZLE_128B) {
  cuuint32_t es[5] = {1, (cuuint32_t)spatial_stride, (cuuint32_t)spatial_stride, 1, 1};
  CUresult r = reinterpret_cast<EncodeTiledFn>(ctx.encode_tiled)(m, dtype, (cuuint32_t)rank, addr, dims, strides,
                                                                box, es, CU_TENSOR_MAP_INTERLEAVE_NONE, swizzle,
                                                                CU_TENSOR_MAP_L2_PROMOTION_L2_256B, CU_TENSOR_MAP_FLOAT_OOB_FILL_NONE);
  if (r != CUDA_SUCCESS) {
    char buf[128];
    snprintf(buf, sizeof buf, "cuTensorMapEncodeTiled failed (CUresult %d, rank %d)", (int)r, rank);
    set_thread_error(buf);
    return 2;
  }
  return 0;
}

void pick_box(int W, int& bw, int& bh, int& bf) {
  if (W % 8 == 0 && W >= 56) { bw = 8; bh = 8; bf = 2; }
  else if (W % 4 == 0) { bw = 4; bh = 4; bf = 8; }
  else if (W % 2 == 0) { bw = 2; bh = 2; bf = 32; }
  else if (W <= 8) { bw = W; bh = 1; bf = BLOCK_M / W; }
  else { bw = 1; bh = 1; bf = 128; }
}

int encode_out(UmmaContext& ctx, CUtensorMap* m, const UmmaConvParams& p, const void* base, int pitch, int n, bool f32) {
  const cuuint64_t es = f32 ? 4 : 2;
  cuuint64_t dims[4] = {(cuuint64_t)n, (cuuint64_t)p.W, (cuuint64_t)p.H, (cuuint64_t)p.F};
  cuuint64_t str[3] = {(cuuint64_t)pitch * es, (cuuint64_t)p.W * pitch * es, (cuuint64_t)p.H * p.W * pitch * es};
  cuuint32_t box[4] = {(cuuint32_t)EPI_COLS, (cuuint32_t)p.bw, (cuuint32_t)p.bh, (cuuint32_t)p.bf};
  return encode(ctx, m, 4, const_cast<void*>(base), dims, str, box, 1, f32 ? CU_TENSOR_MAP_DATA_TYPE_FLOAT32 : CU_TENSOR_MAP_DATA_TYPE_FLOAT16,
                f32 ? CU_TENSOR_MAP_SWIZZLE_64B : CU_TENSOR_MAP_SWIZZLE_32B);
}

int encode_planes(UmmaContext& ctx, CUtensorMap* mhi, CUtensorMap* mlo, const UmmaConvParams& p, const __half* hi, long long lo_off, int pitch, int n) {
  if (int rc = encode_out(ctx, mhi, p, hi, pitch, n, false)) return rc;
  return encode_out(ctx, mlo, p, reinterpret_cast<const char*>(hi) + lo_off, pitch, n, false);
}

int bind_out(UmmaContext& ctx, UmmaConvPlan& plan, View o, float* out32, int n, bool second) {
  UmmaConvParams& p = plan.p;
  CUtensorMap* m = second ? &plan.tmap_o2 : &plan.tmap_o;
  CUtensorMap* mhi = second ? &plan.tmap_o2_hi : &plan.tmap_o_hi;
  CUtensorMap* mlo = second ? &plan.tmap_o2_lo : &plan.tmap_o_lo;
  const bool f32 = p.out_f32 != 0;
  if (int rc = encode_out(ctx, m, p, f32 ? (const void*)(out32 + o.coff) : (const void*)(reinterpret_cast<__half*>(o.base) + o.coff), o.pitch, n, f32))
    return rc;
  *mhi = *m; *mlo = *m;
  const int planes = f32 && o.base;
  if (planes)
    if (int rc = encode_planes(ctx, mhi, mlo, p, reinterpret_cast<__half*>(o.base) + o.coff, o.lo_off, o.pitch, n)) return rc;
  (second ? p.planes2 : p.planes) = planes;
  (second ? p.out2_lo : p.out_lo) = planes ? o.lo_off : 0;
  return 0;
}

int bind_common(UmmaContext& ctx, UmmaConvPlan& plan, View a, View o, int F, int K, int N, int ntaps, const __half* w,
                int a_stride = 1, const UmmaTcOpts* tc = nullptr) {
  plan.enabled = false;
  if (int rc = resolve_encode(ctx)) return rc;
  if (a_stride == 2 || (a_stride == 1 && (a.H != o.H || a.W != o.W))) {
    View ao = a; ao.H = o.H; ao.W = o.W;
    if (int rc = bind_common(ctx, plan, ao, o, F, K, N, ntaps, w, 1, tc)) return rc;
    plan.enabled = false;
    UmmaConvParams& q = plan.p;
    q.a_stride = a_stride;
    cuuint64_t dims[4] = {(cuuint64_t)K, (cuuint64_t)a.W, (cuuint64_t)a.H, (cuuint64_t)F};
    cuuint64_t str[3] = {(cuuint64_t)a.pitch * 2, (cuuint64_t)a.W * a.pitch * 2, (cuuint64_t)a.H * a.W * a.pitch * 2};
    cuuint32_t box[4] = {(cuuint32_t)BLOCK_K, (cuuint32_t)(a_stride * q.bw), (cuuint32_t)(a_stride * q.bh), (cuuint32_t)q.bf};
    if (int rc = encode(ctx, &plan.tmap_a, 4, reinterpret_cast<__half*>(a.base) + a.coff, dims, str, box, a_stride)) return rc;
    plan.tmap_a_lo = plan.tmap_a;
    if (a.lo_off)
      if (int rc = encode(ctx, &plan.tmap_a_lo, 4, reinterpret_cast<__half*>(reinterpret_cast<char*>(a.base) + a.lo_off) + a.coff, dims, str, box, a_stride))
        return rc;
    plan.tmap_a2 = plan.tmap_a; plan.tmap_a2_lo = plan.tmap_a_lo;
    plan.enabled = true;
    return 0;
  }
  if (a.H != o.H || a.W != o.W) { set_thread_error("umma conv: geometry mismatch"); return 1; }
  if (K % 8 || N % 16 || a.pitch % 8 || a.coff % 8 || o.pitch % 8 || o.coff % 8 || ntaps > UMMA_MAX_TAPS) {
    set_thread_error("umma conv: unsupported channel alignment"); return 1; }
  UmmaConvParams& p = plan.p;
  memset(&p, 0, sizeof(p));
  p.W = a.W; p.H = a.H; p.F = F; p.f_direct = 1 << 30;
  pick_box(a.W, p.bw, p.bh, p.bf);
  p.tiles_w = (a.W + p.bw - 1) / p.bw; p.tiles_h = (a.H + p.bh - 1) / p.bh; p.tiles_f = (F + p.bf - 1) / p.bf;
  p.n_tiles = (N + MAX_BLOCK_N - 1) / MAX_BLOCK_N;
  p.block_n = (((N + p.n_tiles - 1) / p.n_tiles) + N_STEP - 1) / N_STEP * N_STEP;
  p.kchunks = (K + BLOCK_K - 1) / BLOCK_K;
  p.K = K;
  p.ntaps = ntaps;
  p.out = reinterpret_cast<__half*>(o.base); p.out_pitch = o.pitch; p.out_coff = o.coff; p.Cout = N;
  p.a_stride = 1; p.mask_y = nullptr; p.mask_pitch = 0; p.mask_coff = 0;
  p.kchunks_a1 = (K + BLOCK_K - 1) / BLOCK_K; p.K1 = K; p.n_split = 1 << 30; p.out2 = p.out; p.out2_pitch = o.pitch; p.out2_coff = o.coff;
  {
    cuuint64_t dims[4] = {(cuuint64_t)K, (cuuint64_t)a.W, (cuuint64_t)a.H, (cuuint64_t)F};
    cuuint64_t str[3] = {(cuuint64_t)a.pitch * 2, (cuuint64_t)a.W * a.pitch * 2, (cuuint64_t)a.H * a.W * a.pitch * 2};
    cuuint32_t box[4] = {(cuuint32_t)BLOCK_K, (cuuint32_t)p.bw, (cuuint32_t)p.bh, (cuuint32_t)p.bf};
    if (int rc = encode(ctx, &plan.tmap_a, 4, reinterpret_cast<__half*>(a.base) + a.coff, dims, str, box)) return rc;
    plan.tmap_a_lo = plan.tmap_a;
    if (a.lo_off)
      if (int rc = encode(ctx, &plan.tmap_a_lo, 4, reinterpret_cast<__half*>(reinterpret_cast<char*>(a.base) + a.lo_off) + a.coff, dims, str, box)) return rc;
  }
  {
    cuuint64_t dims[3] = {(cuuint64_t)K, (cuuint64_t)N, (cuuint64_t)ntaps};
    cuuint64_t str[2] = {(cuuint64_t)K * 2, (cuuint64_t)N * K * 2};
    cuuint32_t box[3] = {(cuuint32_t)BLOCK_K, (cuuint32_t)p.block_n, 1};
    if (int rc = encode(ctx, &plan.tmap_b, 3, const_cast<__half*>(w), dims, str, box)) return rc;
    plan.b_lo_off = tc ? tc->w_lo_off : 0;
    plan.tmap_b_lo = plan.tmap_b;
    if (plan.b_lo_off)
      if (int rc = encode(ctx, &plan.tmap_b_lo, 3, reinterpret_cast<__half*>(reinterpret_cast<char*>(const_cast<__half*>(w)) + plan.b_lo_off), dims, str, box)) return rc;
  }
  plan.tmap_a2 = plan.tmap_a; plan.tmap_a2_lo = plan.tmap_a_lo;
  p.nseg = tc ? 3 : 1; p.out_f32 = tc ? 1 : 0;
  p.stage_bytes = ((A_BYTES + p.block_n * BLOCK_K * 2) * (tc ? 2 : 1) + 1023) / 1024 * 1024;
  p.stages = PIPE_BYTES / p.stage_bytes; if (p.stages > MAX_STAGES) p.stages = MAX_STAGES;
  p.alpha = tc ? tc->alpha : 1.0f; p.alpha_dev = tc ? tc->alpha_dev : nullptr;
  p.mask32 = nullptr; p.mask32_pitch = 0; p.mask32_coff = 0; p.plane_scale = 1.0f; p.flag = nullptr;
  p.out32 = tc ? tc->out32 : nullptr;
  if (tc && (!tc->out32 || !a.lo_off || !tc->w_lo_off)) { set_thread_error("umma conv: split-operand bind needs operand planes and an fp32 output"); return 1; }
  if (int rc = bind_out(ctx, plan, o, p.out32, N, false)) return rc;
  p.out32_2 = p.out32; p.planes2 = p.planes; p.out2_lo = p.out_lo;
  plan.tmap_o2 = plan.tmap_o; plan.tmap_o2_hi = plan.tmap_o_hi; plan.tmap_o2_lo = plan.tmap_o_lo;
  plan.enabled = true;
  return 0;
}

void mark_tc_ok(UmmaConvPlan& plan, int W, bool two_sources) {
  UmmaConvParams& p = plan.p;
  p.tc_ok = 0;
  if (!plan.enabled || p.a_stride != 1) return;
  if (!(p.ntaps == 1 || p.ntaps == 4 || p.ntaps == 9)) return;
  if (p.kchunks_a1 != p.kchunks && (p.ntaps != 1 || !two_sources)) return;
  if (p.out_pitch % 16 || p.out_coff % 16 || p.out2_pitch % 16 || p.out2_coff % 16 || p.n_split % 16 || (p.bias && p.n_tiles * p.block_n > 1024)) return;
  if (W < 7) return;
  p.tc_ok = 1;
}

}

int umma_resolve_encode(UmmaContext& ctx) { return resolve_encode(ctx); }
int umma_encode_f16(UmmaContext& ctx, CUtensorMap* m, int rank, void* addr, const cuuint64_t* dims,
                    const cuuint64_t* strides, const cuuint32_t* box, int spatial_stride) {
  return encode(ctx, m, rank, addr, dims, strides, box, spatial_stride);
}

void umma_context_init(UmmaContext&) {}
void umma_context_destroy(UmmaContext&) {}

int umma_conv_bind_taps(UmmaContext& ctx, UmmaConvPlan& plan, View in, View out, int F, int cin, int cout, int ntaps,
                        const int* dy, const int* dx, const __half* w_tap_n_k, const float* bias, int relu, const UmmaTcOpts* tc, int stride) {
  if (stride != 1 && stride != 2) { set_thread_error("umma conv: stride must be 1 or 2"); return 1; }
  if (int rc = bind_common(ctx, plan, in, out, F, cin, cout, ntaps, w_tap_n_k, stride, tc)) return rc;
  for (int t = 0; t < ntaps; ++t) { plan.p.tap_dy[t] = dy[t]; plan.p.tap_dx[t] = dx[t]; }
  plan.p.bias = bias; plan.p.relu = relu; plan.p.accumulate = 0;
  mark_tc_ok(plan, in.W, false);
  return 0;
}

int umma_conv_bind_fwd(UmmaContext& ctx, UmmaConvPlan& plan, View in, View out, int F, int cin, int cout, int k, int pad,
                       int stride, const __half* w_tap_n_k, const float* bias, const UmmaTcOpts* tc) {
  if (stride != 1 && stride != 2) { set_thread_error("umma conv: stride must be 1 or 2"); return 1; }
  if (int rc = bind_common(ctx, plan, in, out, F, cin, cout, k * k, w_tap_n_k, stride, tc)) return rc;
  for (int r = 0; r < k; ++r)
    for (int s = 0; s < k; ++s) { plan.p.tap_dy[r * k + s] = r - pad; plan.p.tap_dx[r * k + s] = s - pad; }
  plan.p.bias = bias; plan.p.relu = 1; plan.p.accumulate = 0;
  mark_tc_ok(plan, in.W, false);
  return 0;
}

int umma_conv_bind_dgrad(UmmaContext& ctx, UmmaConvPlan& plan, View dz, View dx, int F, int cin, int cout, int k, int pad,
                         const __half* w_tap_k_n, int accumulate, const UmmaTcOpts* tc) {
  if (int rc = bind_common(ctx, plan, dz, dx, F, cout, cin, k * k, w_tap_k_n, 1, tc)) return rc;
  for (int r = 0; r < k; ++r)
    for (int s = 0; s < k; ++s) { plan.p.tap_dy[r * k + s] = pad - r; plan.p.tap_dx[r * k + s] = pad - s; }
  plan.p.bias = nullptr; plan.p.relu = 0; plan.p.accumulate = accumulate;
  mark_tc_ok(plan, dz.W, false);
  return 0;
}

int umma_conv_bind_fused_fwd(UmmaContext& ctx, UmmaConvPlan& plan, View in, View out1, View out2, int F, int cin, int n1, int n2,
                             const __half* w_n_k, const float* bias, const UmmaTcOpts* tc) {
  View o = out1; o.C = n1 + n2;
  if (out1.H != out2.H || out1.W != out2.W || n1 % 16 || n2 % 16 || out2.pitch % 8 || out2.coff % 8) { set_thread_error("fused fwd: bad views"); return 1; }
  if (tc && !tc->out32_2) { set_thread_error("fused fwd: the split-operand bind needs both fp32 destinations"); return 1; }
  if (int rc = bind_common(ctx, plan, in, o, F, cin, n1 + n2, 1, w_n_k, 1, tc)) return rc;
  plan.p.tap_dy[0] = 0; plan.p.tap_dx[0] = 0;
  plan.p.bias = bias; plan.p.relu = 1; plan.p.accumulate = 0;
  plan.p.n_split = n1; plan.p.out2 = reinterpret_cast<__half*>(out2.base); plan.p.out2_pitch = out2.pitch; plan.p.out2_coff = out2.coff;
  if (tc) plan.p.out32_2 = tc->out32_2;
  if (int rc = bind_out(ctx, plan, out1, plan.p.out32, n1, false)) { plan.enabled = false; return rc; }
  if (int rc = bind_out(ctx, plan, out2, plan.p.out32_2, n2, true)) { plan.enabled = false; return rc; }
  mark_tc_ok(plan, in.W, false);
  return 0;
}

int umma_conv_bind_fused_dgrad(UmmaContext& ctx, UmmaConvPlan& plan, View dz1, View dz2, View dx, int F, int cin, int k1, int k2,
                               const __half* w_n_k, int accumulate, const UmmaTcOpts* tc) {
  const int k1p = (k1 + BLOCK_K - 1) / BLOCK_K * BLOCK_K;
  View a = k1 ? dz1 : dz2;
  if (int rc = bind_common(ctx, plan, a, dx, F, k1 ? k1 : k2, cin, 1, w_n_k, 1, tc)) return rc;
  UmmaConvParams& p = plan.p;
  p.tap_dy[0] = 0; p.tap_dx[0] = 0; p.bias = nullptr; p.relu = 0; p.accumulate = accumulate;
  if (k1) {
    if (dz2.H != dz1.H || dz2.W != dz1.W || dz2.pitch % 8 || dz2.coff % 8 || k2 % 8) { set_thread_error("fused dgrad: bad views"); return 1; }
    cuuint64_t dims[4] = {(cuuint64_t)k2, (cuuint64_t)dz2.W, (cuuint64_t)dz2.H, (cuuint64_t)F};
    cuuint64_t str[3] = {(cuuint64_t)dz2.pitch * 2, (cuuint64_t)dz2.W * dz2.pitch * 2, (cuuint64_t)dz2.H * dz2.W * dz2.pitch * 2};
    cuuint32_t box[4] = {(cuuint32_t)BLOCK_K, (cuuint32_t)p.bw, (cuuint32_t)p.bh, (cuuint32_t)p.bf};
    if (int rc = encode(ctx, &plan.tmap_a2, 4, reinterpret_cast<__half*>(dz2.base) + dz2.coff, dims, str, box)) { plan.enabled = false; return rc; }
    p.kchunks_a1 = k1p / BLOCK_K; p.K1 = k1; p.K = k1 + k2;
    p.kchunks = p.kchunks_a1 + (k2 + BLOCK_K - 1) / BLOCK_K;
    cuuint64_t bd[3] = {(cuuint64_t)(k1p + k2), (cuuint64_t)cin, 1};
    cuuint64_t bs[2] = {(cuuint64_t)(k1p + k2) * 2, (cuuint64_t)cin * (k1p + k2) * 2};
    cuuint32_t bb[3] = {(cuuint32_t)BLOCK_K, (cuuint32_t)p.block_n, 1};
    if (int rc = encode(ctx, &plan.tmap_b, 3, const_cast<__half*>(w_n_k), bd, bs, bb)) { plan.enabled = false; return rc; }
    plan.tmap_b_lo = plan.tmap_b;
    if (plan.b_lo_off)
      if (int rc = encode(ctx, &plan.tmap_b_lo, 3, reinterpret_cast<__half*>(reinterpret_cast<char*>(const_cast<__half*>(w_n_k)) + plan.b_lo_off), bd, bs, bb)) {
        plan.enabled = false; return rc; }
    if (tc && !dz2.lo_off) { set_thread_error("fused dgrad: the split-operand bind needs the second source's operand planes"); plan.enabled = false; return 1; }
    plan.tmap_a2_lo = plan.tmap_a2;
    if (dz2.lo_off)
      if (int rc = encode(ctx, &plan.tmap_a2_lo, 4, reinterpret_cast<__half*>(reinterpret_cast<char*>(dz2.base) + dz2.lo_off) + dz2.coff, dims, str, box)) {
        plan.enabled = false; return rc; }
  }
  mark_tc_ok(plan, a.W, k1 != 0);
  return 0;
}

void umma_conv_set_mask(UmmaConvPlan& plan, View y) {
  plan.mask_y = reinterpret_cast<const __half*>(y.base); plan.mask_pitch = y.pitch; plan.mask_coff = y.coff;
}

int umma_conv_set_mask_tc(UmmaContext& ctx, UmmaConvPlan& plan, View y32, View dplanes, float plane_scale, int* flag) {
  if (int rc = encode_planes(ctx, &plan.tmap_mask_hi, &plan.tmap_mask_lo, plan.p, reinterpret_cast<__half*>(dplanes.base) + dplanes.coff, dplanes.lo_off,
                             dplanes.pitch, plan.p.Cout)) return rc;
  plan.mask32 = reinterpret_cast<const float*>(y32.base); plan.mask32_pitch = y32.pitch; plan.mask32_coff = y32.coff;
  plan.mask_planes = true; plan.mask_plane_scale = plane_scale; plan.mask_flag = flag;
  return 0;
}

namespace {
template <int BN, bool DIRECT>
int launch_bn(const UmmaConvPlan& plan, const UmmaConvParams& p, const CUtensorMap& o_hi, const CUtensorMap& o_lo, int grid, cudaStream_t s) {
  static bool attr_set[64] = {};
  auto kern = DIRECT ? umma_conv_tail_kernel<BN> : umma_conv_kernel<BN>;
  int dev = 0;
  cudaGetDevice(&dev);
  if (dev < 0 || dev >= 64 || !attr_set[dev]) {
    if (cudaFuncSetAttribute(kern, cudaFuncAttributeMaxDynamicSharedMemorySize, SMEM_BYTES) != cudaSuccess) {
      set_thread_error("umma conv: cannot raise dynamic shared memory limit"); cudaGetLastError(); return 2; }
    if (dev >= 0 && dev < 64) attr_set[dev] = true;
  }
  kern<<<grid, NUM_THREADS, SMEM_BYTES, s>>>(plan.tmap_a, plan.tmap_a2, plan.tmap_b, plan.tmap_a_lo, plan.tmap_a2_lo, plan.tmap_b_lo, plan.tmap_o, o_hi, o_lo,
                                             plan.tmap_o2, plan.tmap_o2_hi, plan.tmap_o2_lo, p);
  SSNB_LAUNCH_CHECK("umma_conv_kernel");
  return 0;
}
template <int BN>
int launch_bn(const UmmaConvPlan& plan, const UmmaConvParams& p, const CUtensorMap& o_hi, const CUtensorMap& o_lo, int grid, cudaStream_t s) {
  return p.f_direct < (1 << 30) ? launch_bn<BN, true>(plan, p, o_hi, o_lo, grid, s) : launch_bn<BN, false>(plan, p, o_hi, o_lo, grid, s);
}
}

int umma_conv_launch(UmmaContext& ctx, const UmmaConvPlan& plan, cudaStream_t s, bool mask, int frames) {
  if (!plan.enabled) { set_thread_error("umma conv: plan not bound"); return 3; }
  UmmaConvParams p = plan.p;
  if (frames && frames != p.F) {
    if (frames < 1 || frames > p.F || mask || p.accumulate) { set_thread_error("umma conv: a frame count below the plan's runs forward plans only"); return 3; }
    p.F = frames;
    p.tiles_f = (frames + p.bf - 1) / p.bf;
    if (frames % p.bf) p.f_direct = frames - frames % p.bf;
  }
  if (mask && plan.mask_y) { p.mask_y = plan.mask_y; p.mask_pitch = plan.mask_pitch; p.mask_coff = plan.mask_coff; }
  const bool mplanes = mask && p.out_f32 && plan.mask32 && plan.mask_planes;
  if (mplanes) {
    p.mask32 = plan.mask32; p.mask32_pitch = plan.mask32_pitch; p.mask32_coff = plan.mask32_coff;
    p.planes = 1; p.plane_scale = plan.mask_plane_scale; p.flag = plan.mask_flag;
  }
  if (p.out_f32 && p.mask_y) { set_thread_error("umma conv: the fp32 epilogue takes its mask through mask32"); return 3; }
  const CUtensorMap& o_hi = mplanes ? plan.tmap_mask_hi : plan.tmap_o_hi;
  const CUtensorMap& o_lo = mplanes ? plan.tmap_mask_lo : plan.tmap_o_lo;
  const int total = p.tiles_w * p.tiles_h * p.tiles_f * p.n_tiles;
  const int grid = total < ctx.num_sms ? total : ctx.num_sms;
  t_tag.tiles = total; t_tag.block_n = p.block_n;
  switch (p.block_n) {
    case 16: return launch_bn<16>(plan, p, o_hi, o_lo, grid, s);
    case 32: return launch_bn<32>(plan, p, o_hi, o_lo, grid, s);
    case 48: return launch_bn<48>(plan, p, o_hi, o_lo, grid, s);
    case 64: return launch_bn<64>(plan, p, o_hi, o_lo, grid, s);
    case 80: return launch_bn<80>(plan, p, o_hi, o_lo, grid, s);
    case 96: return launch_bn<96>(plan, p, o_hi, o_lo, grid, s);
    case 112: return launch_bn<112>(plan, p, o_hi, o_lo, grid, s);
    case 128: return launch_bn<128>(plan, p, o_hi, o_lo, grid, s);
  }
  set_thread_error("umma conv: unsupported tile width"); return 3;
}

}
```

action-detection_b200/csrc/umma_conv.cuh:

```cuda
#pragma once
#include <cuda.h>
#include <cuda_fp16.h>
#include <cuda_runtime.h>

#include "common.cuh"

namespace ssnb {

constexpr int UMMA_MAX_TAPS = 25;

struct UmmaContext {
  void* encode_tiled = nullptr;
  int num_sms = 132;
};

struct UmmaConvParams {
  int W, H, F;
  int bw, bh, bf;
  int tiles_w, tiles_h, tiles_f;
  int f_direct;
  long long out_lo, out2_lo;
  int n_tiles, block_n;
  int stages, stage_bytes;
  int kchunks, ntaps, K;
  int tap_dy[UMMA_MAX_TAPS], tap_dx[UMMA_MAX_TAPS];
  __half* out; int out_pitch, out_coff, Cout;
  int a_stride;
  const float* bias;
  int relu, accumulate;
  int kchunks_a1, K1;
  int n_split;
  __half* out2; int out2_pitch, out2_coff;
  int tc_ok;
  const __half* mask_y; int mask_pitch, mask_coff;
  int nseg, out_f32;
  float alpha;
  const float* alpha_dev;
  float* out32; int planes;
  float* out32_2; int planes2;
  const float* mask32; int mask32_pitch, mask32_coff;
  float plane_scale; int* flag;
};

struct UmmaConvPlan {
  bool enabled = false;
  const __half* mask_y = nullptr; int mask_pitch = 0, mask_coff = 0;
  CUtensorMap tmap_a, tmap_a2, tmap_b;
  CUtensorMap tmap_a_lo, tmap_a2_lo, tmap_b_lo;
  long long b_lo_off = 0;
  CUtensorMap tmap_o, tmap_o_hi, tmap_o_lo, tmap_o2, tmap_o2_hi, tmap_o2_lo;
  const float* mask32 = nullptr; int mask32_pitch = 0, mask32_coff = 0;
  CUtensorMap tmap_mask_hi, tmap_mask_lo; bool mask_planes = false; float mask_plane_scale = 1.0f; int* mask_flag = nullptr;
  UmmaConvParams p;
};

struct UmmaTcOpts { long long w_lo_off = 0; float* out32 = nullptr; float alpha = 1.0f; const float* alpha_dev = nullptr; float* out32_2 = nullptr; };
void umma_context_init(UmmaContext& ctx);
void umma_context_destroy(UmmaContext& ctx);
int umma_conv_bind_fwd(UmmaContext& ctx, UmmaConvPlan& plan, View in, View out, int F, int cin, int cout, int k, int pad,
                       int stride, const __half* w_tap_n_k, const float* bias, const UmmaTcOpts* tc = nullptr);
int umma_conv_bind_taps(UmmaContext& ctx, UmmaConvPlan& plan, View in, View out, int F, int cin, int cout, int ntaps,
                        const int* dy, const int* dx, const __half* w_tap_n_k, const float* bias, int relu, const UmmaTcOpts* tc = nullptr,
                        int stride = 1);
int umma_conv_bind_dgrad(UmmaContext& ctx, UmmaConvPlan& plan, View dz, View dx, int F, int cin, int cout, int k, int pad,
                         const __half* w_tap_k_n, int accumulate, const UmmaTcOpts* tc = nullptr);
int umma_conv_bind_fused_fwd(UmmaContext& ctx, UmmaConvPlan& plan, View in, View out1, View out2, int F, int cin, int n1, int n2,
                             const __half* w_n_k, const float* bias, const UmmaTcOpts* tc = nullptr);
int umma_conv_bind_fused_dgrad(UmmaContext& ctx, UmmaConvPlan& plan, View dz1, View dz2, View dx, int F, int cin, int k1, int k2,
                               const __half* w_n_k, int accumulate, const UmmaTcOpts* tc = nullptr);
int umma_conv_launch(UmmaContext& ctx, const UmmaConvPlan& plan, cudaStream_t s, bool mask = false, int frames = 0);
void umma_conv_set_mask(UmmaConvPlan& plan, View y);
int umma_conv_set_mask_tc(UmmaContext& ctx, UmmaConvPlan& plan, View y32, View dplanes, float plane_scale, int* flag);

int umma_resolve_encode(UmmaContext& ctx);
int umma_encode_f16(UmmaContext& ctx, CUtensorMap* m, int rank, void* addr, const cuuint64_t* dims,
                    const cuuint64_t* strides, const cuuint32_t* box, int spatial_stride = 1);

struct UmmaWgradParams {
  int W, H, F;
  int bw, bh, bf;
  int tiles_w, tiles_h, tiles_f;
  int ptiles_per_split, splits;
  int ntaps, tap_dy[UMMA_MAX_TAPS], tap_dx[UMMA_MAX_TAPS];
  int Cout, Cin, m_tiles, n_tiles, block_n;
  int x_stride;
  float* bias_partial;
  int taps_per_cta, tap_groups;
  int stages, stage_bytes;
  float* partial;
  int nseg;
  int sub_dh, sub_df;
};
struct UmmaWgradPlan {
  bool enabled = false;
  CUtensorMap tmap_dz, tmap_x;
  CUtensorMap tmap_dz_lo, tmap_x_lo;
  UmmaWgradParams p;
};
constexpr int UMMA_WGRAD_MAX_PTILES = 768;
int umma_wgrad_ptiles(int W, int H, int F);
int umma_wgrad_splits(int ctas, int ptiles, int num_sms, int waves = 1);
int umma_wgrad_bind(UmmaContext& ctx, UmmaWgradPlan& plan, View dz, View x, int F, int cin, int cout, int k, int pad,
                    float* partial, int max_splits, int x_stride = 1);
int umma_wgrad_bind_taps(UmmaContext& ctx, UmmaWgradPlan& plan, View dz, View x, int F, int cin, int cout, int ntaps,
                         const int* dy, const int* dx, float* partial, int max_splits, int x_stride = 1);
int umma_wgrad_launch(UmmaContext& ctx, const UmmaWgradPlan& plan, cudaStream_t s, float* bias_partial = nullptr);

}
```

Before: 823.2.

## Replace zero-upsampled stride-2 dgrad with sub-pixel phase-decomposed convolution

Stride-2 3x3 conv dgrad used to upsample dz into a zero-stuffed buffer and then run a stride-1 conv over it. The new path is a phased conv kernel. It maps each of the 9 taps to one of four output parity phases, loads the dz tile directly via TMA, and accumulates each phase into its own accumulator half. Output is written through four strided tensor maps. This removes the upsample kernel, its workspace traffic and the MMAs over inserted zeros, at the cost of a new kernel variant, extra tensor maps and a tile layout constrained to 2x2 phases.

```diff
diff --git a/action-detection_b200/csrc/common.cuh b/action-detection_b200/csrc/common.cuh
--- a/action-detection_b200/csrc/common.cuh
+++ b/action-detection_b200/csrc/common.cuh
@@ -148,6 +148,5 @@
 int launch_pack_conv1_s2d(const __half* wd, int Cout, int Cin, int Cs, __half* ws, cudaStream_t s);
 int launch_wgrad_finalize_s2d(const float* partial, int splits, int Cout, int Cin, int Cs, const float* mult, float out_scale,
                               const float* unscale, float* dw_ref, int accumulate, cudaStream_t s);
-int launch_upsample2_zero(View src, __half* dst, int H, int W, int F, cudaStream_t s);
 
 }
diff --git a/action-detection_b200/csrc/engine.cu b/action-detection_b200/csrc/engine.cu
--- a/action-detection_b200/csrc/engine.cu
+++ b/action-detection_b200/csrc/engine.cu
@@ -108,7 +108,7 @@
 
 struct ssnb_engine : ssnb::Graph<ssnb::Op> {
   ssnb_config cfg;
-  size_t up_plane = 0, s2d_plane = 0, s2d_w_plane = 0;
+  size_t s2d_plane = 0, s2d_w_plane = 0;
   int* tc_flag = nullptr;
   size_t tc_flag_off = 0;
   float* gscale = nullptr;
@@ -118,7 +118,7 @@
   size_t bn_stat_off = 0, bn_partial_off = 0;
   std::vector<FusedBlock> fused;
   size_t ws_bytes = 0, partial_off = 0, partial_bytes = 0, bpartial_off = 0;
-  size_t s2d_off = 0, s2d_w_off = 0, up_off = 0;
+  size_t s2d_off = 0, s2d_w_off = 0;
   bool fold_pools = true;
   bool s2d_ready = false;
   int Cs = 0;
@@ -319,13 +319,13 @@
     e->s2d_off = operand_region(F * 112 * 112 * 4 * e->Cs * 2, e->s2d_plane);
     e->s2d_w_off = operand_region((size_t)16 * 64 * e->Cs * 2, e->s2d_w_plane);
     if (e->cfg.training) {
-      size_t up = 0;
+      size_t up = 0, up_plane = 0;
       for (const Op& o : e->ops)
         if (o.kind == OP_CONV && o.stride == 2 && o.conv != 0) {
           const Buffer& ib = e->bufs[e->vals[o.in].buf];
           up = std::max(up, F * ib.H * ib.W * (size_t)e->convs[o.conv].cout * 2);
         }
-      e->up_off = operand_region(up, e->up_plane);
+      operand_region(up, up_plane);
       pmax = std::max(pmax, (size_t)e->conv1_tsplits * 16 * 64 * e->Cs * 4);
     }
   }
@@ -440,7 +440,7 @@
                     launch_avgpool3_vec<__half>(dout, din, View(), F, o.grad_accumulate, s));
   }
   const Conv& c = e->convs[o.conv];
-  const View x = e->view(o.in, false), y = e->view(o.out, false), dy = e->view(o.out, true);
+  const View y = e->view(o.out, false), dy = e->view(o.out, true);
   const float* scale = (const float*)(e->ws + e->packed[o.conv].scale);
   float* bpartial = (float*)(e->ws + e->bpartial_off);
   float* dbp = (e->db.size() && e->db[o.conv]) ? e->db[o.conv] : nullptr;
@@ -476,11 +476,6 @@
     }
   }
   if (rc) return rc;
-  if (tc_x && c.stride == 2 && o.conv != 0) {
-    View dz = e->operand(o.out, true);
-    for (int p = 0; p < e->nplanes(); ++p, dz.base = (char*)dz.base + dz.lo_off)
-      if ((rc = launch_upsample2_zero(dz, (__half*)(e->ws + e->up_off + p * e->up_plane), x.H, x.W, F, s))) return rc;
-  }
   if (tc_w) {
     float* partial = (float*)(e->ws + o.partial_off);
     float* bp = bias_w ? (float*)(e->ws + o.bias_partial_off) : nullptr;
@@ -608,13 +603,11 @@
                             c.stride, h->w_fwd(pk), (const float*)(h->ws + pk.bias), h->tc_opts(tf, pk.wplane, h->view(o.out, false).base, 1.0f, pk.wmax));
     if (rc) return h->fail(rc, "bind_fwd(" + c.id + "): " + ssnb::thread_error());
     if (!training) continue;
-    const View in = h->view(o.in, false);
-    View dz = h->operand(o.out, true);
-    if (c.stride == 2) { dz.base = h->ws + h->up_off; dz.H = in.H; dz.W = in.W; dz.C = c.cout; dz.pitch = c.cout; dz.coff = 0; dz.lo_off = (long long)h->up_plane; }
     View dx = h->view(o.in, true);
     const UmmaTcOpts* og = h->tc_opts(tg, pk.wplane, dx.base, 1.0f / gs, pk.wmax);
     if (og) dx.base = nullptr;
-    rc = umma_conv_bind_dgrad(h->umma_ctx, o.umma_dgrad, dz, dx, h->F, c.cin, c.cout, c.kh, c.ph, h->w_dgrad(pk), o.grad_accumulate, og);
+    rc = umma_conv_bind_dgrad(h->umma_ctx, o.umma_dgrad, h->operand(o.out, true), dx, h->F, c.cin, c.cout, c.kh, c.ph, h->w_dgrad(pk),
+                              o.grad_accumulate, og, c.stride);
     if (rc) return h->fail(rc, "bind_dgrad(" + c.id + "): " + ssnb::thread_error());
     tc_gate(o.umma_dgrad);
     if (use_wgrad && (rc = umma_wgrad_bind(h->umma_ctx, o.umma_wgrad, h->operand(o.out, true), h->operand(o.in, false), h->F, c.cin, c.cout,
diff --git a/action-detection_b200/csrc/s2d_glue.cu b/action-detection_b200/csrc/s2d_glue.cu
--- a/action-detection_b200/csrc/s2d_glue.cu
+++ b/action-detection_b200/csrc/s2d_glue.cu
@@ -113,23 +113,6 @@
   }
 }
 
-__global__ void upsample2_zero_kernel(const __half* __restrict__ src, int OH, int OW, int C, int spitch, int scoff,
-                                      __half* __restrict__ dst, int H, int W, int F) {
-  const int G = C / 8;
-  const long long total = (long long)F * H * W * G;
-  const long long i = (long long)blockIdx.x * blockDim.x + threadIdx.x;
-  if (i >= total) return;
-  const unsigned iu = (unsigned)i;
-  const int g = (int)(iu % (unsigned)G);
-  const unsigned pu = iu / (unsigned)G;
-  const int x = (int)(pu % (unsigned)W), y = (int)((pu / (unsigned)W) % (unsigned)H);
-  const long long p = pu;
-  const long long f = pu / (unsigned)(W * H);
-  uint4 v = make_uint4(0u, 0u, 0u, 0u);
-  if (!(x & 1) && !(y & 1) && y / 2 < OH && x / 2 < OW)
-    v = __ldg(reinterpret_cast<const uint4*>(src + ((f * OH + y / 2) * OW + x / 2) * spitch + scoff + g * 8));
-  *reinterpret_cast<uint4*>(dst + p * C + g * 8) = v;
-}
 
 }
 
@@ -169,11 +152,5 @@
   SSNB_LAUNCH_CHECK("wgrad_finalize_s2d_kernel");
   return 0;
 }
-int launch_upsample2_zero(View src, __half* dst, int H, int W, int F, cudaStream_t s) {
-  const long long n = (long long)F * H * W * (src.C / 8);
-  upsample2_zero_kernel<<<(unsigned)((n + 255) / 256), 256, 0, s>>>((const __half*)src.base, src.H, src.W, src.C, src.pitch, src.coff, dst, H, W, F);
-  SSNB_LAUNCH_CHECK("upsample2_zero_kernel");
-  return 0;
-}
 
 }
diff --git a/action-detection_b200/csrc/umma_conv.cu b/action-detection_b200/csrc/umma_conv.cu
--- a/action-detection_b200/csrc/umma_conv.cu
+++ b/action-detection_b200/csrc/umma_conv.cu
@@ -63,18 +63,35 @@
   mma_k<BN, NK>(d0, d1, sa, sb);
 }
 
+template <int BN, int NK>
+__device__ __forceinline__ void mma_block(float* d, uint32_t sa, uint32_t sb, uint32_t b_bytes, bool split) {
+#pragma unroll
+  for (int seg = split ? 0 : 2; seg < 3; ++seg) {
+    const uint32_t a = sa + (seg == 0 ? A_BYTES : 0), b = sb + (seg == 1 ? b_bytes : 0);
+#pragma unroll
+    for (int k = 0; k < NK; ++k) wgmma<BN, 0, 0>(d, make_desc_sw128(a + k * MMA_K * 2), make_desc_sw128(b + k * MMA_K * 2));
+  }
+}
+template <int BN>
+__device__ __forceinline__ void mma_block_nk(int nk, float* d, uint32_t sa, uint32_t sb, uint32_t b_bytes, bool split) {
+  switch (nk) {
+    case 1: mma_block<BN, 1>(d, sa, sb, b_bytes, split); break;
+    case 2: mma_block<BN, 2>(d, sa, sb, b_bytes, split); break;
+    case 3: mma_block<BN, 3>(d, sa, sb, b_bytes, split); break;
+    default: mma_block<BN, BLOCK_K / MMA_K>(d, sa, sb, b_bytes, split); break;
+  }
+}
+
 __device__ __forceinline__ void ring_advance(uint32_t& stage, uint32_t& phase, int n, int stages) {
   const uint32_t s = stage + (uint32_t)n;
   phase ^= (s / (uint32_t)stages) & 1u;
   stage = s % (uint32_t)stages;
 }
 
-template <int BN, bool DIRECT>
+template <int BN, bool DIRECT, bool PH>
 __device__ __forceinline__ void
 umma_conv_body(const CUtensorMap& tmap_a, const CUtensorMap& tmap_a2, const CUtensorMap& tmap_b, const CUtensorMap& tmap_a_lo,
-               const CUtensorMap& tmap_a2_lo, const CUtensorMap& tmap_b_lo, const CUtensorMap& tmap_o, const CUtensorMap& tmap_o_hi,
-               const CUtensorMap& tmap_o_lo, const CUtensorMap& tmap_o2, const CUtensorMap& tmap_o2_hi, const CUtensorMap& tmap_o2_lo,
-               const UmmaConvParams& p) {
+               const CUtensorMap& tmap_a2_lo, const CUtensorMap& tmap_b_lo, const UmmaOutMaps& om, const UmmaConvParams& p) {
   extern __shared__ uint8_t smem_raw[];
   uint8_t* smem = reinterpret_cast<uint8_t*>((reinterpret_cast<uintptr_t>(smem_raw) + 1023) & ~(uintptr_t)1023);
   const int STAGES = p.stages, STAGE_BYTES = p.stage_bytes;
@@ -93,7 +110,7 @@
     asm volatile("prefetch.tensormap [%0];" ::"l"(reinterpret_cast<uint64_t>(&tmap_a)) : "memory");
     asm volatile("prefetch.tensormap [%0];" ::"l"(reinterpret_cast<uint64_t>(&tmap_a2)) : "memory");
     asm volatile("prefetch.tensormap [%0];" ::"l"(reinterpret_cast<uint64_t>(&tmap_b)) : "memory");
-    asm volatile("prefetch.tensormap [%0];" ::"l"(reinterpret_cast<uint64_t>(&tmap_o)) : "memory");
+    asm volatile("prefetch.tensormap [%0];" ::"l"(reinterpret_cast<uint64_t>(&om.o[0])) : "memory");
     for (int i = 0; i < STAGES; ++i) { mbar_init(&full_bar[i], 1); mbar_init(&empty_bar[i], 1); }
     asm volatile("fence.mbarrier_init.release.cluster;" ::: "memory");
   }
@@ -103,7 +120,7 @@
     producer_regs();
     if (threadIdx.x == 0) {
       uint32_t stage = 0, phase = 0;
-      const uint32_t a_bytes = (uint32_t)(p.bw * p.bh * p.bf) * BLOCK_K * 2;
+      const uint32_t a_bytes = (uint32_t)(PH ? 64 : p.bw * p.bh * p.bf) * BLOCK_K * 2;
       const uint32_t tx_bytes = (a_bytes + b_bytes) * nplanes;
       for (int tile = blockIdx.x; tile < total_tiles; tile += gridDim.x) {
         const TileCoord t = decode_tile(p, tile);
@@ -114,7 +131,13 @@
             uint8_t* sb = sa + nplanes * A_BYTES;
             mbar_expect_tx(&full_bar[stage], tx_bytes);
             for (int pl = 0; pl < nplanes; ++pl) {
-              if (kc < p.kchunks_a1)
+              if (PH) {
+                const int ph = p.tap_ph[tap];
+                uint8_t* a0 = sa + pl * A_BYTES + (ph & 2) * 32 * 128;
+                const CUtensorMap* am = pl ? &tmap_a_lo : &tmap_a;
+                tma_load_4d(a0 + (ph & 1) * 32 * 128, am, &full_bar[stage], kc * BLOCK_K, t.w0 / 2 + p.tap_dx[tap], t.h0 / 2 + p.tap_dy[tap], t.f0);
+                tma_load_4d(a0 + (~ph & 1) * 32 * 128, am, &full_bar[stage], kc * BLOCK_K, -64, -64, t.f0);
+              } else if (kc < p.kchunks_a1)
                 tma_load_4d(sa + pl * A_BYTES, pl ? &tmap_a_lo : &tmap_a, &full_bar[stage], kc * BLOCK_K, t.w0 * p.a_stride + p.tap_dx[tap],
                             t.h0 * p.a_stride + p.tap_dy[tap], t.f0);
               else
@@ -153,7 +176,10 @@
         const int kvalid = kc < p.kchunks_a1 ? p.K1 - kc * BLOCK_K : p.K - p.K1 - (kc - p.kchunks_a1) * BLOCK_K;
         const int nk = kvalid >= BLOCK_K ? BLOCK_K / MMA_K : (kvalid + MMA_K - 1) / MMA_K;
         wgmma_fence();
-        switch (nk) {
+        if (PH) {
+          if ((p.tap_blk1 >> (ks / p.kchunks)) & 1) mma_block_nk<BN>(nk, acc[1], sa + 64 * 128, sb, b_bytes, split);
+          else mma_block_nk<BN>(nk, acc[0], sa, sb, b_bytes, split);
+        } else switch (nk) {
           case 1: mma_stage<BN, 1>(acc[0], acc[1], sa, sb, b_bytes, split); break;
           case 2: mma_stage<BN, 2>(acc[0], acc[1], sa, sb, b_bytes, split); break;
           case 3: mma_stage<BN, 3>(acc[0], acc[1], sa, sb, b_bytes, split); break;
@@ -173,13 +199,15 @@
       const bool direct = DIRECT && t.f0 >= p.f_direct;
       bool rv[2][2];
       int rpix[2][2];
+      const int pk = PH ? 2 : 1, sw = p.bw / pk, sh = p.bh / pk, ps = PH ? 5 : 7;
 #pragma unroll
       for (int b = 0; b < 2; ++b)
 #pragma unroll
         for (int h = 0; h < 2; ++h) {
           const int r = b * 64 + warp * 16 + (lane >> 2) + 8 * h;
-          const int rw = r % p.bw, rh = (r / p.bw) % p.bh, rf = r / (p.bw * p.bh);
-          const int w = t.w0 + rw, y = t.h0 + rh, f = t.f0 + rf;
+          const int ph = r >> ps, l = r & ((1 << ps) - 1);
+          const int rw = l % sw, rh = (l / sw) % sh, rf = l / (sw * sh);
+          const int w = t.w0 + pk * rw + (ph & 1), y = t.h0 + pk * rh + (ph >> 1), f = t.f0 + rf;
           rv[b][h] = rf < p.bf && w < p.W && y < p.H && f < p.F;
           rpix[b][h] = (f * p.H + y) * p.W + w;
         }
@@ -341,10 +369,15 @@
         fence_proxy_async_smem();
         named_bar_sync(EPI_BAR + cw, 128);
         if (row == 0 && !direct) {
-          tma_store_4d(d1 ? &tmap_o : &tmap_o2, epi, cd, t.w0, t.h0, t.f0);
-          if (planes) {
-            tma_store_4d(d1 ? &tmap_o_hi : &tmap_o2_hi, epi + EPI_F32_BYTES, cd, t.w0, t.h0, t.f0);
-            tma_store_4d(d1 ? &tmap_o_lo : &tmap_o2_lo, epi + EPI_F32_BYTES + EPI_F16_BYTES, cd, t.w0, t.h0, t.f0);
+          const int rb = p.out_f32 ? 64 : 32, x0 = PH ? t.w0 >> 1 : t.w0, y0 = PH ? t.h0 >> 1 : t.h0;
+#pragma unroll 1
+          for (int q = 0; q < (PH ? 4 : 1); ++q) {
+            const int i = PH ? q : (d1 ? 0 : 1);
+            tma_store_4d(&om.o[i], epi + q * 32 * rb, cd, x0, y0, t.f0);
+            if (planes) {
+              tma_store_4d(&om.hi[i], epi + EPI_F32_BYTES + q * 32 * 32, cd, x0, y0, t.f0);
+              tma_store_4d(&om.lo[i], epi + EPI_F32_BYTES + EPI_F16_BYTES + q * 32 * 32, cd, x0, y0, t.f0);
+            }
           }
           bulk_commit();
         }
@@ -380,16 +413,16 @@
 #define UMMA_CONV_PARAMS                                                                                                    \
   const __grid_constant__ CUtensorMap tmap_a, const __grid_constant__ CUtensorMap tmap_a2, const __grid_constant__ CUtensorMap tmap_b, \
       const __grid_constant__ CUtensorMap tmap_a_lo, const __grid_constant__ CUtensorMap tmap_a2_lo,                               \
-      const __grid_constant__ CUtensorMap tmap_b_lo, const __grid_constant__ CUtensorMap tmap_o,                                   \
-      const __grid_constant__ CUtensorMap tmap_o_hi, const __grid_constant__ CUtensorMap tmap_o_lo,                                \
-      const __grid_constant__ CUtensorMap tmap_o2, const __grid_constant__ CUtensorMap tmap_o2_hi,                                 \
-      const __grid_constant__ CUtensorMap tmap_o2_lo, const __grid_constant__ UmmaConvParams p
-#define UMMA_CONV_ARGS tmap_a, tmap_a2, tmap_b, tmap_a_lo, tmap_a2_lo, tmap_b_lo, tmap_o, tmap_o_hi, tmap_o_lo, tmap_o2, tmap_o2_hi, tmap_o2_lo, p
+      const __grid_constant__ CUtensorMap tmap_b_lo, const __grid_constant__ UmmaOutMaps om,                                       \
+      const __grid_constant__ UmmaConvParams p
+#define UMMA_CONV_ARGS tmap_a, tmap_a2, tmap_b, tmap_a_lo, tmap_a2_lo, tmap_b_lo, om, p
 
 template <int BN>
-__global__ void __launch_bounds__(NUM_THREADS, 1) umma_conv_kernel(UMMA_CONV_PARAMS) { umma_conv_body<BN, false>(UMMA_CONV_ARGS); }
+__global__ void __launch_bounds__(NUM_THREADS, 1) umma_conv_kernel(UMMA_CONV_PARAMS) { umma_conv_body<BN, false, false>(UMMA_CONV_ARGS); }
 template <int BN>
-__global__ void __launch_bounds__(NUM_THREADS, 1) umma_conv_tail_kernel(UMMA_CONV_PARAMS) { umma_conv_body<BN, true>(UMMA_CONV_ARGS); }
+__global__ void __launch_bounds__(NUM_THREADS, 1) umma_conv_phase_kernel(UMMA_CONV_PARAMS) { umma_conv_body<BN, false, true>(UMMA_CONV_ARGS); }
+template <int BN>
+__global__ void __launch_bounds__(NUM_THREADS, 1) umma_conv_tail_kernel(UMMA_CONV_PARAMS) { umma_conv_body<BN, true, false>(UMMA_CONV_ARGS); }
 
 typedef CUresult (*EncodeTiledFn)(CUtensorMap*, CUtensorMapDataType, cuuint32_t, void*, const cuuint64_t*, const cuuint64_t*,
                                   const cuuint32_t*, const cuuint32_t*, CUtensorMapInterleave, CUtensorMapSwizzle,
@@ -436,32 +469,36 @@
   else { bw = 1; bh = 1; bf = 128; }
 }
 
-int encode_out(UmmaContext& ctx, CUtensorMap* m, const UmmaConvParams& p, const void* base, int pitch, int n, bool f32) {
-  const cuuint64_t es = f32 ? 4 : 2;
-  cuuint64_t dims[4] = {(cuuint64_t)n, (cuuint64_t)p.W, (cuuint64_t)p.H, (cuuint64_t)p.F};
-  cuuint64_t str[3] = {(cuuint64_t)pitch * es, (cuuint64_t)p.W * pitch * es, (cuuint64_t)p.H * p.W * pitch * es};
-  cuuint32_t box[4] = {(cuuint32_t)EPI_COLS, (cuuint32_t)p.bw, (cuuint32_t)p.bh, (cuuint32_t)p.bf};
-  return encode(ctx, m, 4, const_cast<void*>(base), dims, str, box, 1, f32 ? CU_TENSOR_MAP_DATA_TYPE_FLOAT32 : CU_TENSOR_MAP_DATA_TYPE_FLOAT16,
+int encode_out(UmmaContext& ctx, CUtensorMap* m, const UmmaConvParams& p, const void* base, int pitch, int n, bool f32, int ph = 0) {
+  const cuuint64_t es = f32 ? 4 : 2, k = p.phased ? 2 : 1;
+  const cuuint64_t W = p.W, H = p.H;
+  const char* at = reinterpret_cast<const char*>(base) + ((ph >> 1) * W + (ph & 1)) * pitch * es;
+  cuuint64_t dims[4] = {(cuuint64_t)n, W / k, H / k, (cuuint64_t)p.F};
+  cuuint64_t str[3] = {k * pitch * es, k * W * pitch * es, H * W * pitch * es};
+  cuuint32_t box[4] = {(cuuint32_t)EPI_COLS, (cuuint32_t)(p.bw / k), (cuuint32_t)(p.bh / k), (cuuint32_t)p.bf};
+  return encode(ctx, m, 4, const_cast<char*>(at), dims, str, box, 1, f32 ? CU_TENSOR_MAP_DATA_TYPE_FLOAT32 : CU_TENSOR_MAP_DATA_TYPE_FLOAT16,
                 f32 ? CU_TENSOR_MAP_SWIZZLE_64B : CU_TENSOR_MAP_SWIZZLE_32B);
 }
 
-int encode_planes(UmmaContext& ctx, CUtensorMap* mhi, CUtensorMap* mlo, const UmmaConvParams& p, const __half* hi, long long lo_off, int pitch, int n) {
-  if (int rc = encode_out(ctx, mhi, p, hi, pitch, n, false)) return rc;
-  return encode_out(ctx, mlo, p, reinterpret_cast<const char*>(hi) + lo_off, pitch, n, false);
+int encode_planes(UmmaContext& ctx, CUtensorMap* mhi, CUtensorMap* mlo, const UmmaConvParams& p, const __half* hi, long long lo_off, int pitch, int n,
+                  int ph = 0) {
+  if (int rc = encode_out(ctx, mhi, p, hi, pitch, n, false, ph)) return rc;
+  return encode_out(ctx, mlo, p, reinterpret_cast<const char*>(hi) + lo_off, pitch, n, false, ph);
 }
 
 int bind_out(UmmaContext& ctx, UmmaConvPlan& plan, View o, float* out32, int n, bool second) {
   UmmaConvParams& p = plan.p;
-  CUtensorMap* m = second ? &plan.tmap_o2 : &plan.tmap_o;
-  CUtensorMap* mhi = second ? &plan.tmap_o2_hi : &plan.tmap_o_hi;
-  CUtensorMap* mlo = second ? &plan.tmap_o2_lo : &plan.tmap_o_lo;
   const bool f32 = p.out_f32 != 0;
-  if (int rc = encode_out(ctx, m, p, f32 ? (const void*)(out32 + o.coff) : (const void*)(reinterpret_cast<__half*>(o.base) + o.coff), o.pitch, n, f32))
-    return rc;
-  *mhi = *m; *mlo = *m;
   const int planes = f32 && o.base;
-  if (planes)
-    if (int rc = encode_planes(ctx, mhi, mlo, p, reinterpret_cast<__half*>(o.base) + o.coff, o.lo_off, o.pitch, n)) return rc;
+  for (int s = 0; s < (p.phased ? 4 : 1); ++s) {
+    const int i = second ? 1 : s;
+    CUtensorMap* m = &plan.out.o[i];
+    if (int rc = encode_out(ctx, m, p, f32 ? (const void*)(out32 + o.coff) : (const void*)(reinterpret_cast<__half*>(o.base) + o.coff), o.pitch, n, f32, s))
+      return rc;
+    plan.out.hi[i] = *m; plan.out.lo[i] = *m;
+    if (planes)
+      if (int rc = encode_planes(ctx, &plan.out.hi[i], &plan.out.lo[i], p, reinterpret_cast<__half*>(o.base) + o.coff, o.lo_off, o.pitch, n, s)) return rc;
+  }
   (second ? p.planes2 : p.planes) = planes;
   (second ? p.out2_lo : p.out_lo) = planes ? o.lo_off : 0;
   return 0;
@@ -534,7 +571,7 @@
   if (tc && (!tc->out32 || !a.lo_off || !tc->w_lo_off)) { set_thread_error("umma conv: split-operand bind needs operand planes and an fp32 output"); return 1; }
   if (int rc = bind_out(ctx, plan, o, p.out32, N, false)) return rc;
   p.out32_2 = p.out32; p.planes2 = p.planes; p.out2_lo = p.out_lo;
-  plan.tmap_o2 = plan.tmap_o; plan.tmap_o2_hi = plan.tmap_o_hi; plan.tmap_o2_lo = plan.tmap_o_lo;
+  for (int i = 1; i < 4; ++i) { plan.out.o[i] = plan.out.o[0]; plan.out.hi[i] = plan.out.hi[0]; plan.out.lo[i] = plan.out.lo[0]; }
   plan.enabled = true;
   return 0;
 }
@@ -583,7 +620,34 @@
 }
 
 int umma_conv_bind_dgrad(UmmaContext& ctx, UmmaConvPlan& plan, View dz, View dx, int F, int cin, int cout, int k, int pad,
-                         const __half* w_tap_k_n, int accumulate, const UmmaTcOpts* tc) {
+                         const __half* w_tap_k_n, int accumulate, const UmmaTcOpts* tc, int stride) {
+  if (stride == 2) {
+    if (k != 3 || pad != 1 || dx.H != 2 * dz.H || dx.W != 2 * dz.W) { set_thread_error("umma conv: a stride-2 data gradient needs k 3, pad 1, even dx"); return 1; }
+    View ag = dz; ag.H = dx.H; ag.W = dx.W;
+    if (int rc = bind_common(ctx, plan, ag, dx, F, cout, cin, 9, w_tap_k_n, 1, tc)) return rc;
+    UmmaConvParams& p = plan.p;
+    if (p.bw % 2 || p.bh % 2 || p.bw * p.bh * p.bf != BLOCK_M) { plan.enabled = false; set_thread_error("umma conv: no phase sub-boxes for this width"); return 1; }
+    cuuint64_t dims[4] = {(cuuint64_t)cout, (cuuint64_t)dz.W, (cuuint64_t)dz.H, (cuuint64_t)F};
+    cuuint64_t str[3] = {(cuuint64_t)dz.pitch * 2, (cuuint64_t)dz.W * dz.pitch * 2, (cuuint64_t)dz.H * dz.W * dz.pitch * 2};
+    cuuint32_t box[4] = {(cuuint32_t)BLOCK_K, (cuuint32_t)(p.bw / 2), (cuuint32_t)(p.bh / 2), (cuuint32_t)p.bf};
+    if (int rc = encode(ctx, &plan.tmap_a, 4, reinterpret_cast<__half*>(dz.base) + dz.coff, dims, str, box)) { plan.enabled = false; return rc; }
+    plan.tmap_a_lo = plan.tmap_a;
+    if (dz.lo_off)
+      if (int rc = encode(ctx, &plan.tmap_a_lo, 4, reinterpret_cast<__half*>(reinterpret_cast<char*>(dz.base) + dz.lo_off) + dz.coff, dims, str, box)) {
+        plan.enabled = false; return rc; }
+    plan.tmap_a2 = plan.tmap_a; plan.tmap_a2_lo = plan.tmap_a_lo;
+    for (int t = 0; t < 9; ++t) {
+      const int r = t / 3, c = t % 3, a = (r + 1) % 2, b = (c + 1) % 2;
+      p.tap_ph[t] = 2 * a + b; p.tap_dy[t] = (a + 1 - r) / 2; p.tap_dx[t] = (b + 1 - c) / 2;
+      p.tap_blk1 |= (uint32_t)a << t;
+    }
+    p.phased = 1;
+    p.bias = nullptr; p.relu = 0; p.accumulate = accumulate;
+    if (int rc = bind_out(ctx, plan, dx, p.out32, cin, false)) { plan.enabled = false; return rc; }
+    mark_tc_ok(plan, dx.W, false);
+    return 0;
+  }
+  if (stride != 1) { set_thread_error("umma conv: stride must be 1 or 2"); return 1; }
   if (int rc = bind_common(ctx, plan, dz, dx, F, cout, cin, k * k, w_tap_k_n, 1, tc)) return rc;
   for (int r = 0; r < k; ++r)
     for (int s = 0; s < k; ++s) { plan.p.tap_dy[r * k + s] = pad - r; plan.p.tap_dx[r * k + s] = pad - s; }
@@ -646,18 +710,24 @@
 }
 
 int umma_conv_set_mask_tc(UmmaContext& ctx, UmmaConvPlan& plan, View y32, View dplanes, float plane_scale, int* flag) {
-  if (int rc = encode_planes(ctx, &plan.tmap_mask_hi, &plan.tmap_mask_lo, plan.p, reinterpret_cast<__half*>(dplanes.base) + dplanes.coff, dplanes.lo_off,
-                             dplanes.pitch, plan.p.Cout)) return rc;
+  for (int s = 0; s < 4; ++s) {
+    if (s == 0 || plan.p.phased) {
+      if (int rc = encode_planes(ctx, &plan.mask_hi[s], &plan.mask_lo[s], plan.p, reinterpret_cast<__half*>(dplanes.base) + dplanes.coff,
+                                 dplanes.lo_off, dplanes.pitch, plan.p.Cout, s)) return rc;
+    } else {
+      plan.mask_hi[s] = plan.mask_hi[0]; plan.mask_lo[s] = plan.mask_lo[0];
+    }
+  }
   plan.mask32 = reinterpret_cast<const float*>(y32.base); plan.mask32_pitch = y32.pitch; plan.mask32_coff = y32.coff;
   plan.mask_planes = true; plan.mask_plane_scale = plane_scale; plan.mask_flag = flag;
   return 0;
 }
 
 namespace {
-template <int BN, bool DIRECT>
-int launch_bn(const UmmaConvPlan& plan, const UmmaConvParams& p, const CUtensorMap& o_hi, const CUtensorMap& o_lo, int grid, cudaStream_t s) {
+template <int BN, bool DIRECT, bool PH>
+int launch_bn(const UmmaConvPlan& plan, const UmmaConvParams& p, const UmmaOutMaps& om, int grid, cudaStream_t s) {
   static bool attr_set[64] = {};
-  auto kern = DIRECT ? umma_conv_tail_kernel<BN> : umma_conv_kernel<BN>;
+  auto kern = DIRECT ? umma_conv_tail_kernel<BN> : PH ? umma_conv_phase_kernel<BN> : umma_conv_kernel<BN>;
   int dev = 0;
   cudaGetDevice(&dev);
   if (dev < 0 || dev >= 64 || !attr_set[dev]) {
@@ -665,14 +735,14 @@
       set_thread_error("umma conv: cannot raise dynamic shared memory limit"); cudaGetLastError(); return 2; }
     if (dev >= 0 && dev < 64) attr_set[dev] = true;
   }
-  kern<<<grid, NUM_THREADS, SMEM_BYTES, s>>>(plan.tmap_a, plan.tmap_a2, plan.tmap_b, plan.tmap_a_lo, plan.tmap_a2_lo, plan.tmap_b_lo, plan.tmap_o, o_hi, o_lo,
-                                             plan.tmap_o2, plan.tmap_o2_hi, plan.tmap_o2_lo, p);
+  kern<<<grid, NUM_THREADS, SMEM_BYTES, s>>>(plan.tmap_a, plan.tmap_a2, plan.tmap_b, plan.tmap_a_lo, plan.tmap_a2_lo, plan.tmap_b_lo, om, p);
   SSNB_LAUNCH_CHECK("umma_conv_kernel");
   return 0;
 }
 template <int BN>
-int launch_bn(const UmmaConvPlan& plan, const UmmaConvParams& p, const CUtensorMap& o_hi, const CUtensorMap& o_lo, int grid, cudaStream_t s) {
-  return p.f_direct < (1 << 30) ? launch_bn<BN, true>(plan, p, o_hi, o_lo, grid, s) : launch_bn<BN, false>(plan, p, o_hi, o_lo, grid, s);
+int launch_bn(const UmmaConvPlan& plan, const UmmaConvParams& p, const UmmaOutMaps& om, int grid, cudaStream_t s) {
+  if (p.phased) return launch_bn<BN, false, true>(plan, p, om, grid, s);
+  return p.f_direct < (1 << 30) ? launch_bn<BN, true, false>(plan, p, om, grid, s) : launch_bn<BN, false, false>(plan, p, om, grid, s);
 }
 }
 
@@ -680,7 +750,7 @@
   if (!plan.enabled) { set_thread_error("umma conv: plan not bound"); return 3; }
   UmmaConvParams p = plan.p;
   if (frames && frames != p.F) {
-    if (frames < 1 || frames > p.F || mask || p.accumulate) { set_thread_error("umma conv: a frame count below the plan's runs forward plans only"); return 3; }
+    if (frames < 1 || frames > p.F || mask || p.accumulate || p.phased) { set_thread_error("umma conv: a frame count below the plan's runs forward plans only"); return 3; }
     p.F = frames;
     p.tiles_f = (frames + p.bf - 1) / p.bf;
     if (frames % p.bf) p.f_direct = frames - frames % p.bf;
@@ -692,20 +762,24 @@
     p.planes = 1; p.plane_scale = plan.mask_plane_scale; p.flag = plan.mask_flag;
   }
   if (p.out_f32 && p.mask_y) { set_thread_error("umma conv: the fp32 epilogue takes its mask through mask32"); return 3; }
-  const CUtensorMap& o_hi = mplanes ? plan.tmap_mask_hi : plan.tmap_o_hi;
-  const CUtensorMap& o_lo = mplanes ? plan.tmap_mask_lo : plan.tmap_o_lo;
+  UmmaOutMaps mom;
+  if (mplanes) {
+    mom = plan.out;
+    for (int i = 0; i < 4; ++i) { mom.hi[i] = plan.mask_hi[i]; mom.lo[i] = plan.mask_lo[i]; }
+  }
+  const UmmaOutMaps& om = mplanes ? mom : plan.out;
   const int total = p.tiles_w * p.tiles_h * p.tiles_f * p.n_tiles;
   const int grid = total < ctx.num_sms ? total : ctx.num_sms;
   t_tag.tiles = total; t_tag.block_n = p.block_n;
   switch (p.block_n) {
-    case 16: return launch_bn<16>(plan, p, o_hi, o_lo, grid, s);
-    case 32: return launch_bn<32>(plan, p, o_hi, o_lo, grid, s);
-    case 48: return launch_bn<48>(plan, p, o_hi, o_lo, grid, s);
-    case 64: return launch_bn<64>(plan, p, o_hi, o_lo, grid, s);
-    case 80: return launch_bn<80>(plan, p, o_hi, o_lo, grid, s);
-    case 96: return launch_bn<96>(plan, p, o_hi, o_lo, grid, s);
-    case 112: return launch_bn<112>(plan, p, o_hi, o_lo, grid, s);
-    case 128: return launch_bn<128>(plan, p, o_hi, o_lo, grid, s);
+    case 16: return launch_bn<16>(plan, p, om, grid, s);
+    case 32: return launch_bn<32>(plan, p, om, grid, s);
+    case 48: return launch_bn<48>(plan, p, om, grid, s);
+    case 64: return launch_bn<64>(plan, p, om, grid, s);
+    case 80: return launch_bn<80>(plan, p, om, grid, s);
+    case 96: return launch_bn<96>(plan, p, om, grid, s);
+    case 112: return launch_bn<112>(plan, p, om, grid, s);
+    case 128: return launch_bn<128>(plan, p, om, grid, s);
   }
   set_thread_error("umma conv: unsupported tile width"); return 3;
 }
diff --git a/action-detection_b200/csrc/umma_conv.cuh b/action-detection_b200/csrc/umma_conv.cuh
--- a/action-detection_b200/csrc/umma_conv.cuh
+++ b/action-detection_b200/csrc/umma_conv.cuh
@@ -24,6 +24,8 @@
   int stages, stage_bytes;
   int kchunks, ntaps, K;
   int tap_dy[UMMA_MAX_TAPS], tap_dx[UMMA_MAX_TAPS];
+  int phased, tap_ph[UMMA_MAX_TAPS];
+  unsigned tap_blk1;
   __half* out; int out_pitch, out_coff, Cout;
   int a_stride;
   const float* bias;
@@ -42,15 +44,17 @@
   float plane_scale; int* flag;
 };
 
+struct UmmaOutMaps { CUtensorMap o[4], hi[4], lo[4]; };
+
 struct UmmaConvPlan {
   bool enabled = false;
   const __half* mask_y = nullptr; int mask_pitch = 0, mask_coff = 0;
   CUtensorMap tmap_a, tmap_a2, tmap_b;
   CUtensorMap tmap_a_lo, tmap_a2_lo, tmap_b_lo;
   long long b_lo_off = 0;
-  CUtensorMap tmap_o, tmap_o_hi, tmap_o_lo, tmap_o2, tmap_o2_hi, tmap_o2_lo;
+  UmmaOutMaps out;
   const float* mask32 = nullptr; int mask32_pitch = 0, mask32_coff = 0;
-  CUtensorMap tmap_mask_hi, tmap_mask_lo; bool mask_planes = false; float mask_plane_scale = 1.0f; int* mask_flag = nullptr;
+  CUtensorMap mask_hi[4], mask_lo[4]; bool mask_planes = false; float mask_plane_scale = 1.0f; int* mask_flag = nullptr;
   UmmaConvParams p;
 };
 
@@ -63,7 +67,7 @@
                         const int* dy, const int* dx, const __half* w_tap_n_k, const float* bias, int relu, const UmmaTcOpts* tc = nullptr,
                         int stride = 1);
 int umma_conv_bind_dgrad(UmmaContext& ctx, UmmaConvPlan& plan, View dz, View dx, int F, int cin, int cout, int k, int pad,
-                         const __half* w_tap_k_n, int accumulate, const UmmaTcOpts* tc = nullptr);
+                         const __half* w_tap_k_n, int accumulate, const UmmaTcOpts* tc = nullptr, int stride = 1);
 int umma_conv_bind_fused_fwd(UmmaContext& ctx, UmmaConvPlan& plan, View in, View out1, View out2, int F, int cin, int n1, int n2,
                              const __half* w_n_k, const float* bias, const UmmaTcOpts* tc = nullptr);
 int umma_conv_bind_fused_dgrad(UmmaContext& ctx, UmmaConvPlan& plan, View dz1, View dz2, View dx, int F, int cin, int k1, int k2,
```

After: 829.7 (median of 6 runs). Within noise of the previous version (+0.8%).
